# mohammadasim98/mv-ldm

Measured on AMD Instinct MI355X. Metric: denoised views/sec @ 256x256, 4 views, 50 DDIM steps, higher is better.
Workload: dtype bf16

## Files before the change

mv_ldm_amd/_build.py:

```python
from __future__ import annotations

import json
import os
import re
import subprocess
import sys
from concurrent.futures import ThreadPoolExecutor
from pathlib import Path

CSRC = Path(__file__).resolve().parent / "csrc"
LIB = CSRC / "libmvldm_hip.so"
SOURCES = ["api.cpp", "plan.cpp", "igemm.hip", "igemm_small.hip", "igemm_large.hip", "igemm_xl.hip", "igemm_halo.hip", "pack.hip", "attention.hip", "norm.hip", "misc.hip",
           "wgrad.hip", "attention_bwd.hip", "norm_bwd.hip", "train_misc.hip", "linear_pp.hip", "linear_pw.hip", "linear_ws.hip", "linear_rs.hip", "skinny.hip", "metrics.hip", "lpips.hip"]
HEADERS = [*sorted(CSRC.glob("*.h")), CSRC.parent.parent / "include" / "mvldm.h"]
FLAGS = ["--offload-arch=gfx950", "-O3", "-std=c++17", "-fPIC", "-ffp-contract=off", "-Wno-unused-result",
         "-Rpass-analysis=kernel-resource-usage"]
RES = CSRC / "kernel_resources.json"


def _hipcc() -> str:
    for c in (os.environ.get("HIPCC"), "/opt/rocm/bin/hipcc", "hipcc"):
        if c and (os.path.isabs(c) and os.path.exists(c) or not os.path.isabs(c)):
            return c
    raise RuntimeError("hipcc not found")


def _stale(target: Path, deps) -> bool:
    if not target.exists():
        return True
    t = target.stat().st_mtime
    return any(Path(d).stat().st_mtime > t for d in deps)


def build(force: bool = False, verbose: bool = False) -> Path:
    hipcc = _hipcc()
    flags = list(FLAGS)
    if os.environ.get("MVLDM_EXPERIMENTS") == "1":
        flags.append("-DMVLDM_EXPERIMENTS")
    objs, jobs = [], []
    for src in SOURCES:
        s = CSRC / src
        o = CSRC / (s.stem + ".o")
        objs.append(o)
        if force or _stale(o, [s, *HEADERS]):
            cmd = [hipcc, *flags, "-x", "hip", "-c", str(s), "-o", str(o)]
            jobs.append(cmd)
    if jobs:
        def run(cmd):
            if verbose:
                print(" ".join(cmd), flush=True)
            r = subprocess.run(cmd, capture_output=True, text=True)
            if r.returncode:
                raise RuntimeError(f"hipcc failed: {' '.join(cmd)}\n{r.stdout}\n{r.stderr}")
            Path(cmd[-1]).with_suffix(".res.json").write_text(json.dumps(_resources(r.stderr), indent=0))
        with ThreadPoolExecutor(max_workers=min(8, len(jobs))) as ex:
            list(ex.map(run, jobs))
    if force or jobs or _stale(LIB, objs):
        cmd = [hipcc, "--offload-arch=gfx950", "-shared", "-fPIC", "-o", str(LIB), *map(str, objs)]
        r = subprocess.run(cmd, capture_output=True, text=True)
        if r.returncode:
            raise RuntimeError(f"link failed:\n{r.stdout}\n{r.stderr}")
    parts = [o.with_suffix(".res.json") for o in objs]
    if all(q.exists() for q in parts) and (not RES.exists() or _stale(RES, parts)):
        merged = {}
        for q in parts:
            merged.update(json.loads(q.read_text()))
        RES.write_text(json.dumps(merged, indent=0, sort_keys=True))
    return LIB


_FIELDS = {"VGPRs": "vgpr", "AGPRs": "agpr", "TotalSGPRs": "sgpr", "ScratchSize [bytes/lane]": "scratch", "VGPRs Spill": "vgpr_spill",
           "Occupancy [waves/SIMD]": "waves_per_simd"}


def _resources(stderr: str) -> dict:
    out, cur = {}, None
    for line in stderr.splitlines():
        m = re.search(r"remark:\s+(.*?)\s*\[-Rpass-analysis", line)
        if not m:
            continue
        body = m.group(1)
        if body.startswith("Function Name:"):
            cur = out.setdefault(body.split(":", 1)[1].strip(), {})
        elif cur is not None and ":" in body:
            k, v = body.rsplit(":", 1)
            if k.strip() in _FIELDS and v.strip().lstrip("-").isdigit():
                cur[_FIELDS[k.strip()]] = int(v)
    return out


if __name__ == "__main__":
    print(build(force="--force" in sys.argv, verbose=True))
```

mv_ldm_amd/csrc/igemm.hip:

```cpp
#include <algorithm>
#include <cstdio>
#include <cstdlib>

#include "igemm_common.h"

namespace mvldm {

template <typename T> __global__ __launch_bounds__(256) void igemm_splitk_reduce(const IgemmParams p) {
    const bool geglu = p.epilogue == MVLDM_EPI_GEGLU;
    const size_t total = (size_t)p.M * p.n_dst;
    const size_t slab = (size_t)p.M * p.n_pad;
    for (size_t idx = (size_t)blockIdx.x * 256 + threadIdx.x; idx < total; idx += (size_t)gridDim.x * 256) {
        const int m = (int)(idx / p.n_dst), col = (int)(idx - (size_t)m * p.n_dst);
        float v;
        if (geglu) {
            const int nv = (col >> 5) * 64 + (col & 31), ng = nv + 32;
            float a = 0.f, g = 0.f;
            for (int s = 0; s < p.splitk; ++s) {
                a += p.ws[s * slab + (size_t)m * p.n_pad + nv];
                g += p.ws[s * slab + (size_t)m * p.n_pad + ng];
            }
            if (p.bias) { a += p.bias[col]; g += p.bias[p.n_dst + col]; }
            v = a * gelu_erf_fast(g);
        } else {
            float a = 0.f;
            for (int s = 0; s < p.splitk; ++s) a += p.ws[s * slab + (size_t)m * p.n_pad + col];
            if (p.bias) a += p.bias[col];
            if (p.row_bias) a += p.row_bias[(size_t)(m / p.hw_out) * p.row_bias_ld + col];
            if (p.epilogue == MVLDM_EPI_SILU) a = silu_f(a);
            else if (p.epilogue == MVLDM_EPI_GELU) a = gelu_erf_fast(a);
            v = a;
        }
        epilogue_store<T, true>(p, m, col, v);
    }
}

template <typename T> __global__ __launch_bounds__(256) void igemm_splitk_reduce_vec(const IgemmParams p) {
    const bool geglu = p.epilogue == MVLDM_EPI_GEGLU;
    const int cpr = p.n_dst / 8;
    const size_t total = (size_t)p.M * cpr;
    const size_t slab = (size_t)p.M * p.n_pad;
    for (size_t idx = (size_t)blockIdx.x * 256 + threadIdx.x; idx < total; idx += (size_t)gridDim.x * 256) {
        const int m = (int)(idx / cpr), col = (int)(idx - (size_t)m * cpr) * 8;
        const int nv = geglu ? (col >> 5) * 64 + (col & 31) : col;
        const float* w0 = p.ws + (size_t)m * p.n_pad + nv;
        float a[8], g[8];
#pragma unroll
        for (int e = 0; e < 8; ++e) a[e] = g[e] = 0.f;
        int s = 0;
        for (; s + 4 <= p.splitk; s += 4) {
            f32x4 lo[4], hi[4], gl[4], gh[4];
#pragma unroll
            for (int u = 0; u < 4; ++u) {
                lo[u] = *reinterpret_cast<const f32x4*>(w0 + (s + u) * slab);
                hi[u] = *reinterpret_cast<const f32x4*>(w0 + (s + u) * slab + 4);
                if (geglu) {
                    gl[u] = *reinterpret_cast<const f32x4*>(w0 + (s + u) * slab + 32);
                    gh[u] = *reinterpret_cast<const f32x4*>(w0 + (s + u) * slab + 36);
                }
            }
#pragma unroll
            for (int u = 0; u < 4; ++u) {
#pragma unroll
                for (int e = 0; e < 4; ++e) { a[e] += lo[u][e]; a[4 + e] += hi[u][e]; }
                if (geglu) {
#pragma unroll
                    for (int e = 0; e < 4; ++e) { g[e] += gl[u][e]; g[4 + e] += gh[u][e]; }
                }
            }
        }
        for (; s < p.splitk; ++s) {
            const f32x4 lo = *reinterpret_cast<const f32x4*>(w0 + s * slab), hi = *reinterpret_cast<const f32x4*>(w0 + s * slab + 4);
#pragma unroll
            for (int e = 0; e < 4; ++e) { a[e] += lo[e]; a[4 + e] += hi[e]; }
            if (geglu) {
                const f32x4 gl = *reinterpret_cast<const f32x4*>(w0 + s * slab + 32), gh = *reinterpret_cast<const f32x4*>(w0 + s * slab + 36);
#pragma unroll
                for (int e = 0; e < 4; ++e) { g[e] += gl[e]; g[4 + e] += gh[e]; }
            }
        }
        if (p.bias) {
#pragma unroll
            for (int e = 0; e < 8; ++e) a[e] += p.bias[col + e];
        }
        if (geglu) {
#pragma unroll
            for (int e = 0; e < 8; ++e) a[e] *= gelu_erf_fast(g[e] + (p.bias ? p.bias[p.n_dst + col + e] : 0.f));
        } else {
            if (p.row_bias) {
                const float* rb = p.row_bias + (size_t)(m / p.hw_out) * p.row_bias_ld + col;
#pragma unroll
                for (int e = 0; e < 8; ++e) a[e] += rb[e];
            }
            if (p.epilogue == MVLDM_EPI_SILU) {
#pragma unroll
                for (int e = 0; e < 8; ++e) a[e] = silu_f(a[e]);
            } else if (p.epilogue == MVLDM_EPI_GELU) {
#pragma unroll
                for (int e = 0; e < 8; ++e) a[e] = gelu_erf_fast(a[e]);
            }
        }
#pragma unroll
        for (int e = 0; e < 8; ++e) a[e] *= p.out_scale;
        if (p.residual) {
            const Chunk<T> rc = load_chunk<T>(reinterpret_cast<const T*>(p.residual) + (size_t)m * p.n_dst + col);
#pragma unroll
            for (int e = 0; e < 8; ++e) a[e] += rc.get(e);
        }
        size_t drow = (size_t)m;
        if (p.scatter) {
            const int img = m / p.hw_out, rem = m - img * p.hw_out;
            const int i = rem / p.w_out, j = rem - i * p.w_out;
            drow = ((size_t)img * (2 * p.h_out) + 2 * i + p.ph_y) * (size_t)(2 * p.w_out) + 2 * j + p.ph_x;
        }
        Chunk<T> oc;
#pragma unroll
        for (int e = 0; e < 8; ++e) oc.set(e, a[e]);
        store_chunk<T>(reinterpret_cast<T*>(p.dst) + drow * p.dst_ld + col, oc);
    }
}

static int env_int(const char* name, int dflt) { return knob_int(name, dflt); }
static const int kEnvTarget = env_int("MVLDM_IGEMM_TARGET", 0);
static const int kEnvSync = env_int("MVLDM_IGEMM_SYNC", 0);
static const int kEnvPx = env_int("MVLDM_IGEMM_PX", 0);
static const int kEnvNoStage = env_int("MVLDM_IGEMM_NOSTAGE", 0);
#ifdef MVLDM_EXPERIMENTS
static const int kEnvFake = env_int("MVLDM_IGEMM_FAKE", 0);
#else
static constexpr int kEnvFake = 0;
#endif

static thread_local int t_force_sync = 0;

static int launch_igemm(const IgemmParams& p, int tile, int act_dtype, hipStream_t s) {
    if (tile >= 1 && tile <= 5) return igemm_launch_small(p, tile, act_dtype, s);
    if (tile >= 6 && tile <= 8) return igemm_launch_large(p, tile, act_dtype, s);
    if (tile == 9 || tile == 10 || tile == 18) return igemm_launch_xl(p, tile, act_dtype, s);
    if (tile == 11 || tile == 17) return igemm_launch_halo(p, tile, act_dtype, s);
    return set_error(MVLDM_ERR_ARG, "igemm: bad tile %d", tile);
}


static void choose_config(const mvldm_igemm_desc& d, int M, int k_tiles, int& tile, int& splitk, size_t ws_bytes) {
    const int target = kEnvTarget ? kEnvTarget : 512;
    if (tile == 0) {
        const bool can10 = d.act_dtype != MVLDM_F32 && d.k_order == 1 && d.dst_dtype != MVLDM_F32 && d.n_pad % 320 == 0 &&
                           d.epilogue != MVLDM_EPI_GEGLU && d.upsample != 1 && d.n_out % 8 == 0 && (d.dst_ld <= 0 || d.dst_ld % 8 == 0) &&
                           !(d.ksize == 3 && d.src1);
        const int wgs10 = cdiv(M, 256) * (d.n_pad / 320);
        const double eff10 = (double)wgs10 / (256.0 * cdiv(wgs10, 256));
        if (can10 && (wgs10 >= 1024 || (wgs10 >= 512 && (eff10 >= 0.9 || d.ksize == 1)))) tile = 10;
        else if (M <= 32) tile = 5;
        else if (M <= 64) tile = 4;
        else if (d.ksize >= 2) tile = cdiv(M, 256) * cdiv(d.n_pad, 128) >= 300 ? 7 : 2;
        else if (d.n_pad >= 768 && d.act_dtype != MVLDM_F32 && d.k_order == 1 && d.dst_dtype != MVLDM_F32 &&
                 cdiv(M, 256) * cdiv(d.n_pad, 256) >= 1024)
            tile = 9;
        else if (d.k_pad >= 1024 && d.n_pad >= 1024 && cdiv(M, 128) * cdiv(d.n_pad, 256) >= 300) tile = 8;
        else tile = d.n_pad < 640 ? 2 : 3;
    }
    const int tm = cdiv(M, kTiles[tile].bm), tn = cdiv(d.n_pad, kTiles[tile].bn);
    if (splitk == 0) {
        splitk = 1;
        const int wgs = tm * tn;
        if (wgs < target) splitk = std::min(std::max(k_tiles / 4, 1), cdiv(target, wgs));
        if (d.workspace == nullptr) splitk = 1;
        while (splitk > 1 && (size_t)splitk * M * d.n_pad * sizeof(float) > ws_bytes) --splitk;
    }
    splitk = std::max(1, std::min(splitk, k_tiles));
}

static int fill_params(const mvldm_igemm_desc& d, IgemmParams& p, int& tile) {
    const int epc = d.act_dtype == MVLDM_F32 ? 4 : 8;
    const int bk = d.act_dtype == MVLDM_F32 ? 32 : 64;
    MVLDM_REQUIRE(d.src0 && d.weight && d.dst, "igemm: null pointer");
    const bool phase = d.upsample >= 2;
    MVLDM_REQUIRE(d.upsample >= 0 && d.upsample <= 5, "igemm: upsample %d", d.upsample);
    MVLDM_REQUIRE(phase ? (d.ksize == 2 && d.stride == 1 && d.h_out == d.h_in && d.w_out == d.w_in && !d.src1 && !d.residual &&
                           !d.row_bias && d.act_dtype != MVLDM_F32 && d.dst_dtype == d.act_dtype && d.k_order == 1)
                        : (d.ksize == 1 || d.ksize == 3),
                  "igemm: ksize %d / upsample %d", d.ksize, d.upsample);
    MVLDM_REQUIRE(d.stride == 1 || d.stride == 2, "igemm: stride %d", d.stride);
    MVLDM_REQUIRE(d.c0 % epc == 0 && d.c1 % epc == 0 && d.c0 > 0, "igemm: channels (%d,%d) must be multiples of %d", d.c0, d.c1, epc);
    MVLDM_REQUIRE((d.c1 == 0) == (d.src1 == nullptr), "igemm: src1/c1 mismatch");
    MVLDM_REQUIRE(d.k_pad % bk == 0 && d.k_pad >= d.ksize * d.ksize * (d.c0 + d.c1), "igemm: k_pad %d", d.k_pad);
    MVLDM_REQUIRE(d.n_pad % 64 == 0 && d.n_pad >= d.n_out, "igemm: n_pad %d (n_out %d)", d.n_pad, d.n_out);
    MVLDM_REQUIRE(d.dst_dtype == d.act_dtype || d.dst_dtype == MVLDM_F32, "igemm: dst dtype");
    if (d.epilogue == MVLDM_EPI_GEGLU)
        MVLDM_REQUIRE(d.n_out % 64 == 0 && !d.row_bias, "igemm: GEGLU needs n_out %% 64 == 0");
    p.src0 = d.src0; p.src1 = d.src1; p.weight = d.weight; p.bias = d.bias; p.row_bias = d.row_bias;
    p.residual = d.residual; p.dst = d.dst; p.ws = d.workspace;
    p.c0 = d.c0; p.c1 = d.c1; p.ctot = d.c0 + d.c1;
    p.n_img = d.n_img; p.h_in = d.h_in; p.w_in = d.w_in; p.h_out = d.h_out; p.w_out = d.w_out;
    p.hw_out = d.h_out * d.w_out;
    p.ksize = d.ksize; p.stride = d.stride; p.pad = d.pad; p.upsample = phase ? 0 : d.upsample; p.taps = d.ksize * d.ksize;
    p.scatter = phase; p.ph_y = phase ? (d.upsample - 2) >> 1 : 0; p.ph_x = phase ? (d.upsample - 2) & 1 : 0;
    p.ty0 = phase ? p.ph_y - 1 : -d.pad; p.tx0 = phase ? p.ph_x - 1 : -d.pad;
    p.cy = phase ? 1 - p.ph_y : d.ksize / 2; p.cx = phase ? 1 - p.ph_x : d.ksize / 2;
    p.M = d.n_img * p.hw_out; p.n_out = d.n_out; p.n_pad = d.n_pad; p.k_pad = d.k_pad;
    p.n_dst = d.epilogue == MVLDM_EPI_GEGLU ? d.n_out / 2 : d.n_out;
    p.rb_vec = d.row_bias && ((uintptr_t)d.row_bias % 16 == 0) && d.row_bias_ld % 4 == 0;
    p.bias_vec = d.bias && ((uintptr_t)d.bias % 16 == 0);
    p.row_bias_ld = d.row_bias_ld; p.epilogue = d.epilogue; p.dst_f32 = d.dst_dtype == MVLDM_F32;
    p.out_scale = d.out_scale;
    p.dst_ld = d.dst_ld > 0 ? d.dst_ld : p.n_dst;
    MVLDM_REQUIRE(p.dst_ld >= p.n_dst, "igemm: dst_ld %d < n_dst %d", p.dst_ld, p.n_dst);
    p.k_tiles = d.k_pad / bk;
    tile = d.tile & 63;
    t_force_sync = (d.tile >> 12) & 1;
    const int force_px = (d.tile >> 8) & 15;
    int splitk = d.splitk;
    MVLDM_REQUIRE(((tile >= 0 && tile <= kNumTiles) || tile == 17 || deep_tile(tile)) && splitk >= 0, "igemm: tile/splitk");
    choose_config(d, p.M, p.k_tiles, tile, splitk, d.workspace_bytes);
    if (splitk > 1)
        MVLDM_REQUIRE(d.workspace && (size_t)splitk * p.M * d.n_pad * sizeof(float) <= d.workspace_bytes,
                      "igemm: split-K workspace too small");
    const double es = 2.0;
    const double b0 = (double)d.n_img * d.h_in * d.w_in * d.c0 * es, b1 = (double)d.n_img * d.h_in * d.w_in * d.c1 * es;
    const double bw = (double)d.n_pad * d.k_pad * es;
    p.use_bl = d.act_dtype != MVLDM_F32 && d.k_order == 1 && !t_force_sync && !kEnvSync &&
               b0 < 4.0e9 && b1 < 4.0e9 && bw < 4.0e9;
    if (d.act_dtype != MVLDM_F32 && d.k_order == 1 && !t_force_sync && !kEnvSync && !p.use_bl) {
        static bool warned = false;
        if (!warned) {
            warned = true;
            fprintf(stderr, "[mvldm] igemm: operand of %.2f GB exceeds the 4 GB range of the fast 16-bit loop; using the slower "
                            "64-bit-address loop (split the batch to avoid this)\n", std::max(std::max(b0, b1), bw) / 1e9);
        }
    }
    p.src0_bytes = (unsigned)b0; p.src1_bytes = (unsigned)b1; p.w_bytes = (unsigned)bw;
    p.fake = kEnvFake;
    p.nt_store = stream_stores((size_t)p.M * (size_t)p.n_dst * (p.dst_f32 || d.act_dtype == MVLDM_F32 ? 4 : 2));
    if (kEnvFake & 1) p.src0_bytes = p.src1_bytes = 0;
    if (kEnvFake & 2) p.w_bytes = 0;
    if (tile >= 6 && !p.use_bl) tile = 2;
    if (deep_tile(tile) && d.upsample) tile = 2;
    p.splitk = splitk;
    if (p.use_bl) {
        const int cbs = p.k_tiles / p.taps;
        const int per = cdiv(cbs, std::min(splitk, cbs));
        p.k_tiles_per_split = per * p.taps;
        p.splitk = cdiv(cbs, per);
    } else {
        p.k_tiles_per_split = cdiv(p.k_tiles, splitk);
        p.splitk = cdiv(p.k_tiles, p.k_tiles_per_split);
    }
    p.stage_epi = d.act_dtype != MVLDM_F32 && !kEnvNoStage && (p.splitk > 1 || (!p.dst_f32 && p.n_dst % 8 == 0 && p.dst_ld % 8 == 0));
    if (tile >= 9 && tile <= 10 && (!p.stage_epi || (tile == 10 && d.epilogue == MVLDM_EPI_GEGLU))) tile = 7;
    if (tile == 11 && !(p.use_bl && p.stage_epi && p.splitk == 1 && d.ksize == 3 && d.stride == 1 && d.pad == 1 && !d.upsample &&
                        d.h_out == d.h_in && d.w_out == d.w_in && halo_rows_for(d.w_in) <= 384 && halo_smem(d.w_in) <= 160 * 1024))
        tile = 7;
    if (tile == 17 && !(p.use_bl && p.stage_epi && p.splitk == 1 && d.ksize == 3 && d.stride == 1 && d.pad == 1 && !d.upsample && d.c1 == 0 &&
                        d.h_out == d.h_in && d.w_out == d.w_in && d.epilogue != MVLDM_EPI_GEGLU && halow_smem(d.w_in) <= 160 * 1024))
        tile = 7;
    if (phase) {
        MVLDM_REQUIRE(p.use_bl && p.stage_epi, "igemm: 2x2 phase conv needs the lean 16-bit loop and an 8-aligned 16-bit output");
        if (tile != 7 && tile != 10) tile = 2;
    }
    if (p.use_bl && d.upsample == 1 && tile != 7) tile = 2;
    if (p.use_bl && d.upsample != 1) {
        const int hc = (d.h_out - 1) * d.stride + p.ty0 + p.cy, wc = (d.w_out - 1) * d.stride + p.tx0 + p.cx;
        MVLDM_REQUIRE(p.ty0 + p.cy >= 0 && p.tx0 + p.cx >= 0 && hc < d.h_in && wc < d.w_in,
                      "igemm: conv geometry (pad %d, stride %d) not supported", d.pad, d.stride);
    }
    p.tiles_m = cdiv(p.M, kTiles[tile].bm);
    p.tiles_n = cdiv(d.n_pad, kTiles[tile].bn);
    p.korder = d.k_order;
    if (d.k_order)
        MVLDM_REQUIRE(d.k_order == 1 && p.ctot % bk == 0 && d.c0 % bk == 0 && d.k_pad == p.taps * p.ctot,
                      "igemm: k_order 1 needs channel counts (%d,%d) multiples of %d", d.c0, d.c1, bk);
    {
        const double a_bytes = (double)d.n_img * d.h_in * d.w_in * p.ctot, w_bytes = (double)d.n_pad * d.k_pad;
        double best = 1e300;
        for (int px = 1; px <= 8; px *= 2) {
            const int py = 8 / px;
            const int sm = cdiv(p.tiles_m, px), sn = cdiv(p.tiles_n, py);
            const double waste = (double)(8 * sm * sn) / ((double)p.tiles_m * p.tiles_n);
            const double cost = (py * a_bytes + px * w_bytes) * waste * waste;
            if (cost < best) { best = cost; p.px = px; p.sub_m = sm; p.sub_n = sn; }
        }
        p.m_fast = w_bytes >= a_bytes;
        const int fpx = force_px ? force_px : kEnvPx;
        if (fpx > 0 && fpx <= 8 && (8 % fpx) == 0) {
            p.px = fpx; p.sub_m = cdiv(p.tiles_m, p.px); p.sub_n = cdiv(p.tiles_n, 8 / p.px);
        }
        p.grp_m = p.grp_n = 1;
        static const int kGroup = knob_int("MVLDM_IGEMM_GROUP", -1);
        if (kGroup != 0 && ((tile >= 7 && tile <= 10) || tile == 17) && p.sub_m * p.sub_n > 32) {
            const double ax = a_bytes / p.px, wx = w_bytes / (8 / p.px);
            double bestc = 1e300;
            for (int gm = 1; gm <= 32; gm *= 2) {
                if (kGroup > 0 && gm != kGroup) continue;
                const int gme = std::min(gm, p.sub_m), gne = std::min(32 / gm, p.sub_n);
                const double c = ax * cdiv(p.sub_n, gne) + wx * cdiv(p.sub_m, gme);
                if (c < bestc) { bestc = c; p.grp_m = gme; p.grp_n = gne; }
            }
        }
    }
    return MVLDM_OK;
}

int linear_pp_run(const mvldm_igemm_desc& d, hipStream_t s);
int linear_pw_run(const mvldm_igemm_desc& d, hipStream_t s);
int linear_ws_run(const mvldm_igemm_desc& d, hipStream_t s);
int skinny_run(const mvldm_igemm_desc& d, hipStream_t s);
int linear_rs_run(const mvldm_igemm_desc& d, hipStream_t s);

int igemm_run(const mvldm_igemm_desc& d, hipStream_t s) {
    IgemmParams p;
    int tile = 0;
    if (d.n_img == 0 || d.h_out == 0 || d.w_out == 0) return MVLDM_OK;
    const int req = d.tile & 63;
    if (req == 15) return skinny_run(d, s);
    if (req == 12 || req == 13 || req == 14 || req == 19) {
        MVLDM_REQUIRE(d.src0 && d.weight && d.dst, "igemm: null pointer");
        return req == 12 ? linear_pp_run(d, s) : req == 13 ? linear_pw_run(d, s) : req == 14 ? linear_ws_run(d, s) : linear_rs_run(d, s);
    }
    MVLDM_REQUIRE(d.k_order != 2, "igemm: the fragment-order pack (k_order 2) is read by tile 15 only");
    int rc = fill_params(d, p, tile);
    if (rc) return rc;
    if (p.M == 0) return MVLDM_OK;
    rc = dispatch_dtype(d.act_dtype, [&](auto t) {
        using T = decltype(t);
        int r = launch_igemm(p, tile, Elt<T>::DT, s);
        if (r) return r;
        if (p.splitk > 1) {
            if constexpr (sizeof(T) == 2) {
                if (!p.dst_f32 && p.n_dst % 8 == 0 && p.dst_ld % 8 == 0 && ((uintptr_t)p.ws % 16) == 0 &&
                    (!p.residual || ((uintptr_t)p.residual % 16) == 0) && ((uintptr_t)p.dst % 16) == 0) {
                    const size_t chunks = (size_t)p.M * (p.n_dst / 8);
                    hipLaunchKernelGGL(igemm_splitk_reduce_vec<T>, dim3((unsigned)std::min<size_t>((chunks + 255) / 256, 4096)), dim3(256), 0, s, p);
                    return check_launch();
                }
            }
            const size_t total = (size_t)p.M * p.n_dst;
            const int blocks = (int)std::min<size_t>((total + 255) / 256, 4096);
            hipLaunchKernelGGL(igemm_splitk_reduce<T>, dim3(blocks), dim3(256), 0, s, p);
            return check_launch();
        }
        return (int)MVLDM_OK;
    });
    return rc;
}

}

using namespace mvldm;

extern "C" int mvldm_igemm_fwd(const mvldm_igemm_desc* d, mvldm_stream_t stream) {
    MVLDM_REQUIRE(d != nullptr, "igemm: null desc");
    return igemm_run(*d, (hipStream_t)stream);
}

extern "C" size_t mvldm_igemm_workspace_bytes(const mvldm_igemm_desc* d) {
    if (!d) return 0;
    const size_t M = (size_t)d->n_img * d->h_out * d->w_out;
    return (size_t)16 * M * d->n_pad * sizeof(float);
}
```

mv_ldm_amd/csrc/linear_pw.hip:

```cpp
#include <cstdlib>

#include "linear_common.h"

namespace mvldm {

struct LinPWParams {
    const void* a; const void* a1; const void* w; const float* bias; const void* residual; void* dst;
    int M, K, c0, c1, kt0, n_out, n_pad, n_dst, dst_ld, k_steps;
    int tiles_m, tiles_n, m_per;
    int gm, gn, nbn, wgx;
    int nt_store, touch;
    int spread;
    float out_scale;
    unsigned a_bytes, a1_bytes, w_bytes, bias_bytes, res_bytes, dst_bytes;
    unsigned* trace; int trace_blk, trace_wave, trace_stagger;
};

#ifdef MVLDM_PW_TRACE
#define PW_STAMP() if (tr_on && tr_n < 190) { reinterpret_cast<unsigned*>(smem + G::SLAB + 1280)[tr_n++] = (unsigned)__builtin_readcyclecounter(); }
#else
#define PW_STAMP()
#endif

#ifdef MVLDM_EXPERIMENTS
static const int kPwFake = knob_int("MVLDM_PW_FAKE", 0);
#else
static constexpr int kPwFake = 0;
#endif
#ifdef MVLDM_EXPERIMENTS_NOGELU
#define PW_GELU(x) (x)
#else
#define PW_GELU(x) gelu_erf_16(x)
#endif

constexpr int PW_BM = 256, PW_NW = 8;
#ifndef PW_SP3
#define PW_SP3 4
#define PW_SP0 3
#define PW_SP1 2
#endif

template <int TN> struct PwGeo {
    static constexpr int BN = 64 * TN;
    static constexpr int A_SLOT = PW_BM * 128, W_SLOT = BN * 128, STAGE = A_SLOT + W_SLOT;
    static constexpr int A_IT = PW_BM / 8 / PW_NW;
    static constexpr int W_IT = BN / 8 / PW_NW;
    static constexpr int P = A_IT + W_IT;
    static constexpr int Q0 = PW_SP3 < P ? PW_SP3 : P, Q1 = Q0 + PW_SP0 < P ? Q0 + PW_SP0 : P, Q2 = Q1 + PW_SP1 < P ? Q1 + PW_SP1 : P;
    static constexpr int RING = 2 * STAGE;
    static constexpr int SLAB = RING;
    static constexpr int SMEM = SLAB + 2048;
};

struct PwAddr {
    unsigned a0, a1;
    unsigned w;
    int m0, n0;
    bool valid;
};

template <int TN, int LO = 0, int HI = 1 << 20>
__device__ __forceinline__ void pw_issue_a(const LinPWParams& p, char* smem, int slot, int wave, int lane, int ks, const PwAddr& ad) {
    using G = PwGeo<TN>;
    const bool second = ks >= p.kt0;
    const void* abase = second ? p.a1 : p.a;
    const unsigned abytes = second ? p.a1_bytes : p.a_bytes;
    const int c = second ? p.c1 : p.c0;
    const __amdgpu_buffer_rsrc_t ra = __builtin_amdgcn_make_buffer_rsrc(const_cast<void*>(abase), 0, abytes, 0x00020000);
    const int soff = (second ? ks - p.kt0 : ks) * 128;
    char* stage = smem + slot * G::STAGE;
    const unsigned v = second ? ad.a1 : ad.a0;
    const int row = wave * 8 + (lane >> 3);
#pragma unroll
    for (int it = (LO > 0 ? LO : 0); it < (HI < G::A_IT ? HI : G::A_IT); ++it) {
        const unsigned off = (ad.valid && ad.m0 + row + 64 * it < p.M) ? v : kBufOob;
        __builtin_amdgcn_raw_ptr_buffer_load_lds(ra, (__attribute__((address_space(3))) void*)(stage + (wave + PW_NW * it) * 1024), 16, off,
                                                 soff + it * 128 * c, 0, 0);
    }
}
template <int TN, int LO = 0, int HI = 1 << 20>
__device__ __forceinline__ void pw_issue_w(const LinPWParams& p, char* smem, int slot, int wave, int ks, const PwAddr& ad) {
    using G = PwGeo<TN>;
    const __amdgpu_buffer_rsrc_t rw = __builtin_amdgcn_make_buffer_rsrc(const_cast<void*>(p.w), 0, p.w_bytes, 0x00020000);
    const int soff = ks * 128;
    char* stage = smem + slot * G::STAGE + G::A_SLOT;
#pragma unroll
    for (int it = (LO > 0 ? LO : 0); it < (HI < G::W_IT ? HI : G::W_IT); ++it) {
        const unsigned off = (ad.valid && ad.n0 + 64 * it < p.n_pad) ? ad.w : kBufOob;
        __builtin_amdgcn_raw_ptr_buffer_load_lds(rw, (__attribute__((address_space(3))) void*)(stage + (wave + PW_NW * it) * 1024), 16, off,
                                                 soff + it * 128 * p.K, 0, 0);
    }
}

template <int TN, int LO, int HI>
__device__ __forceinline__ void pw_issue_group(const LinPWParams& p, char* smem, int slot, int wave, int lane, int ks, const PwAddr& ad) {
    using G = PwGeo<TN>;
    if constexpr (LO < HI && LO < G::A_IT) pw_issue_a<TN, LO, HI>(p, smem, slot, wave, lane, ks, ad);
    if constexpr (LO < HI && HI > G::A_IT) pw_issue_w<TN, LO - G::A_IT, HI - G::A_IT>(p, smem, slot, wave, ks, ad);
}

template <int TN>
__device__ __forceinline__ void pw_touch_a(const LinPWParams& p, char* smem, int wave, int lane, int tm, int ks, bool valid) {
    using G = PwGeo<TN>;
    const bool second = ks >= p.kt0;
    const void* abase = second ? p.a1 : p.a;
    const unsigned abytes = second ? p.a1_bytes : p.a_bytes;
    const int c = second ? p.c1 : p.c0;
    const __amdgpu_buffer_rsrc_t ra = __builtin_amdgcn_make_buffer_rsrc(const_cast<void*>(abase), 0, abytes, 0x00020000);
    const int m = tm * PW_BM + wave * 32 + (lane >> 1);
    const unsigned off = (valid && m < p.M) ? ((unsigned)m * (unsigned)c * 2u + (unsigned)(lane & 1) * 64u) : kBufOob;
    __builtin_amdgcn_raw_ptr_buffer_load_lds(ra, (__attribute__((address_space(3))) void*)(smem + G::SLAB + 1792), 4, off,
                                             (second ? ks - p.kt0 : ks) * 128, 0, 0);
}

template <int TN>
__device__ __forceinline__ void pw_offsets(const LinPWParams& p, bool valid, int tm, int tn, int wave, int lane, PwAddr& ad) {
    using G = PwGeo<TN>;
    const int slot = lane & 7, rsub = lane >> 3;
    const int row = wave * 8 + rsub;
    const unsigned chunk = (unsigned)((slot ^ ((row >> 1) & 7)) * 8);
    const int m = tm * PW_BM + row, n = tn * G::BN + row;
    ad.a0 = ((unsigned)m * (unsigned)p.c0 + chunk) * 2u;
    ad.a1 = ((unsigned)m * (unsigned)p.c1 + chunk) * 2u;
    ad.w = ((unsigned)n * (unsigned)p.K + chunk) * 2u;
    ad.m0 = tm * PW_BM;
    ad.n0 = tn * G::BN;
    ad.valid = valid;
}

template <int TN>
__device__ __forceinline__ unsigned pw_bias_off(const LinPWParams& p, bool geglu, bool valid, int tn, int t) {
    using G = PwGeo<TN>;
    const int pc = tn * G::BN + 4 * t;
    int oc = pc;
    if (geglu) {
        const int blk = pc >> 5, w = pc & 31;
        oc = ((blk & 1) ? p.n_dst : 0) + (blk >> 1) * 32 + w;
    }
    return (valid && 4 * t < G::BN && pc < p.n_out) ? (unsigned)oc * 4u : kBufOob;
}

template <bool NT>
__device__ __forceinline__ void pw_store2(const u32x4& rdst, const u32x4& d0, unsigned o0, const u32x4& d1, unsigned o1) {
    if constexpr (NT)
        asm volatile("s_nop 4\n\tbuffer_store_dwordx4 %0, %1, %4, 0 offen nt\n\tbuffer_store_dwordx4 %2, %3, %4, 0 offen nt\n\ts_nop 2"
                     ::"v"(d0), "v"(o0), "v"(d1), "v"(o1), "s"(rdst) : "memory");
    else
        asm volatile("s_nop 4\n\tbuffer_store_dwordx4 %0, %1, %4, 0 offen\n\tbuffer_store_dwordx4 %2, %3, %4, 0 offen\n\ts_nop 2"
                     ::"v"(d0), "v"(o0), "v"(d1), "v"(o1), "s"(rdst) : "memory");
}

template <int CTRL> __device__ __forceinline__ u32x4 pw_qperm(const u32x4& v) {
    u32x4 r;
#pragma unroll
    for (int c = 0; c < 4; ++c) r[c] = (unsigned)__builtin_amdgcn_update_dpp(0, (int)v[c], CTRL, 0xF, 0xF, true);
    return r;
}
__device__ __forceinline__ u32x4 pw_sel(bool take_a, const u32x4& a, const u32x4& b) {
    u32x4 r;
#pragma unroll
    for (int c = 0; c < 4; ++c) r[c] = take_a ? a[c] : b[c];
    return r;
}
__device__ __forceinline__ void pw_quad_transpose(u32x4& c0, u32x4& c1, u32x4& c2, u32x4& c3, bool odd, bool upper) {
    constexpr int X1 = 0xB1, X2 = 0x4E;
    const u32x4 x0 = pw_sel(odd, pw_qperm<X1>(c1), c0), x1 = pw_sel(odd, c1, pw_qperm<X1>(c0));
    const u32x4 x2 = pw_sel(odd, pw_qperm<X1>(c3), c2), x3 = pw_sel(odd, c3, pw_qperm<X1>(c2));
    c0 = pw_sel(upper, pw_qperm<X2>(x2), x0);
    c2 = pw_sel(upper, x2, pw_qperm<X2>(x0));
    c1 = pw_sel(upper, pw_qperm<X2>(x3), x1);
    c3 = pw_sel(upper, x3, pw_qperm<X2>(x1));
}
__device__ __forceinline__ unsigned pw_line_off(int M, int tm, int wm, int i, int j, int half, int l31, int hi, int col0, int ld, int n_dst) {
    const int t = 2 * (j & 1) + half, k = l31 & 3;
    const int m = tm * PW_BM + wm * 64 + i * 32 + (l31 & ~3) + t;
    const int col = col0 + 32 * (j & ~1) + 8 * (2 * k + hi);
    return (m < M && col < n_dst) ? ((unsigned)m * (unsigned)ld + (unsigned)col) * 2u : kBufOob;
}

template <typename T, int TN, int EPI, bool RES, bool NT>
__global__ __launch_bounds__(512) void linear_pw_kernel(const LinPWParams p) {
    using G = PwGeo<TN>;
    using Frag = typename LinMma<T>::Frag;
    constexpr bool GEGLU = EPI == MVLDM_EPI_GEGLU;
    static_assert(!GEGLU || TN % 2 == 0, "GEGLU pairs value / gate blocks inside a wave tile");
    static_assert(!(GEGLU && RES), "no caller");
    constexpr int NOUT = GEGLU ? TN / 2 : TN;
    extern __shared__ __attribute__((aligned(16))) char smem[];
    const int tid = threadIdx.x, lane = tid & 63;
    const int wave = __builtin_amdgcn_readfirstlane(tid >> 6);
    const int wm = wave >> 1, wn = wave & 1;
    const int hi = lane >> 5, l31 = lane & 31;
    const int prm = lin_perm(l31);

    const int xcd = blockIdx.x & 7, lid = blockIdx.x >> 3;
    const int m_lo = xcd * p.m_per, m_cnt = min(p.tiles_m, m_lo + p.m_per) - m_lo;
    LinTileIter<LinPWParams> cur, nxt, iss;
    cur.set(p, 0, lid, m_lo, m_cnt);
    if (!cur.valid) return;
    nxt.set(p, cur.r + 1, lid, m_lo, m_cnt);
    iss = cur;

    u32x4 rdst;
    rdst[0] = (unsigned)(uintptr_t)p.dst; rdst[1] = (unsigned)((uintptr_t)p.dst >> 32) & 0xFFFFu; rdst[2] = p.dst_bytes; rdst[3] = 0x00020000u;

    const int a_off = (wm * 64 + l31) * 128 + ((hi ^ ((l31 >> 1) & 7)) << 4);
    const int w_off = G::A_SLOT + (wn * 32 * TN + prm) * 128 + ((hi ^ ((prm >> 1) & 7)) << 4);

    f32x16 acc[2][TN];
    PwAddr ad;
    int ks_i = 1;
    const int kT = p.k_steps;

#ifdef MVLDM_PW_TRACE
    for (int i = 0; i < (lid & 3) * p.trace_stagger; ++i) __builtin_amdgcn_s_sleep(8);
#endif
    {
        pw_offsets<TN>(p, true, cur.tm, cur.tn, wave, lane, ad);
#pragma unroll
        for (int g = 0; g < 2; ++g) {
            pw_issue_a<TN>(p, smem, g, wave, lane, g, ad);
            pw_issue_w<TN>(p, smem, g, wave, g, ad);
        }
        const u32x4 b = lin_load_bias<G::BN>(p, GEGLU, true, cur.tn, tid);
        __builtin_amdgcn_s_waitcnt(waitcnt_vmcnt(0));
        if (4 * tid < G::BN) *reinterpret_cast<u32x4*>(smem + G::SLAB + tid * 16) = b;
    }
    int rs = 0;
#ifdef MVLDM_PW_TRACE
    const bool tr_on = p.trace && (int)blockIdx.x == p.trace_blk && wave == p.trace_wave;
    int tr_n = 0;
#endif

#define PW_SUB(ca_, cw_, na_, nw_, NEXT_, nslot_, nkk_, MODE_, SPN_)                                              \
    {                                                                                                             \
        const char* st_ = smem + (nslot_) * G::STAGE;                                                             \
        const int ao_ = a_off ^ ((nkk_) << 5), wo_ = w_off ^ ((nkk_) << 5);                                       \
        if (NEXT_) {                                                                                              \
            na_[0] = lin_frag<T>(st_ + ao_);                                                                      \
            na_[1] = lin_frag<T>(st_ + ao_ + 4096);                                                               \
            nw_[0] = lin_frag<T>(st_ + wo_);                                                                      \
        }                                                                                                         \
        _Pragma("unroll") for (int j = 0; j < TN; ++j) {                                                          \
            __builtin_amdgcn_sched_barrier(0);                                                                    \
            acc[0][j] = LinMma<T>::mma(cw_[j], ca_[0], acc[0][j]);                                                \
            acc[1][j] = LinMma<T>::mma(cw_[j], ca_[1], acc[1][j]);                                                \
            if (NEXT_ && j + 1 < TN) nw_[j + 1] = lin_frag<T>(st_ + wo_ + (j + 1) * 4096);                        \
            if ((MODE_) == 1 && j == 0) {                                                                         \
                if (++ks_i == kT) {                                                                               \
                    ks_i = 0;                                                                                     \
                    iss.set(p, iss.r + 1, lid, m_lo, m_cnt);                                                  \
                    pw_offsets<TN>(p, iss.valid, iss.tm, iss.tn, wave, lane, ad);                                 \
                }                                                                                                 \
                if (SPN_) pw_issue_group<TN, 0, G::Q0>(p, smem, rs, wave, lane, ks_i, ad);                        \
                else pw_issue_a<TN>(p, smem, rs, wave, lane, ks_i, ad);                                           \
            }                                                                                                     \
            if ((MODE_) == 1 && j == 2 && !(SPN_)) pw_issue_w<TN>(p, smem, rs, wave, ks_i, ad);                   \
            if ((MODE_) == 2 && j == 1 && pend) pw_issue_group<TN, G::Q0, G::Q1>(p, smem, rs ^ 1, wave, lane, ks_i, ad); \
            if ((MODE_) == 3 && j == 1 && pend) pw_issue_group<TN, G::Q1, G::Q2>(p, smem, rs ^ 1, wave, lane, ks_i, ad); \
            if ((MODE_) == 4 && j == 1 && pend) pw_issue_group<TN, G::Q2, G::P>(p, smem, rs ^ 1, wave, lane, ks_i, ad);  \
        }                                                                                                         \
        __builtin_amdgcn_sched_barrier(0);                                                                        \
    }
#define PW_STEP(LAST_, WAIT_, TOUCH_, SPN_)                                                                       \
    {                                                                                                             \
        PW_STAMP()                                                                                                \
        if ((TOUCH_) && p.touch) {                                                                                \
             \
            const int kt_ = ks_t + PW_TOUCH_AHEAD;                                                                \
            const bool own_ = kt_ < kT;                                                                           \
            pw_touch_a<TN>(p, smem, wave, lane, __builtin_amdgcn_readfirstlane(own_ ? cur.tm : nxt.tm),           \
                           __builtin_amdgcn_readfirstlane(own_ ? kt_ : kt_ - kT), own_ || nxt.valid);             \
        }                                                                                                         \
        PW_SUB(fa0, fw0, fa1, fw1, true, rs, 1, 2, false)                                                         \
        PW_SUB(fa1, fw1, fa0, fw0, true, rs, 2, 3, false)                                                         \
        PW_SUB(fa0, fw0, fa1, fw1, true, rs, 3, 4, false)                                                         \
        PW_STAMP()                                                                                                \
        if ((TOUCH_) && p.touch) __builtin_amdgcn_s_waitcnt(kWaitStep1);                                          \
        else __builtin_amdgcn_s_waitcnt(WAIT_);                                                                   \
        PW_STAMP()                                                                                                \
        __builtin_amdgcn_s_barrier();                                                                             \
        PW_STAMP()                                                                                                \
        {                                                                                                         \
            const bool spn_ = (SPN_);                                                                             \
            PW_SUB(fa1, fw1, fa0, fw0, !(LAST_), rs ^ 1, 0, 1, spn_)                                              \
            pend = spn_;                                                                                          \
        }                                                                                                         \
        rs ^= 1;                                                                                                  \
    }
    bool pend = false;
    const bool sp = p.spread && !p.touch && kT >= 4;
    Frag fa0[2], fw0[TN], fa1[2], fw1[TN];
    constexpr int kWaitLds = 0xC07F;
    constexpr int kWaitFirst = waitcnt_vmcnt(4 * NOUT) & ~0x0F00;
    constexpr int kWaitStepT = waitcnt_vmcnt(0) & ~0x0F00;
    constexpr int kWaitStep1 = waitcnt_vmcnt(1) & ~0x0F00;
    constexpr int PW_TOUCH_AHEAD = 4;

    for (; cur.valid; cur = nxt, nxt.set(p, nxt.r + 1, lid, m_lo, m_cnt)) {
        __builtin_amdgcn_s_barrier();
        {
            const float* slab = reinterpret_cast<const float*>(smem + G::SLAB) + wn * 32 * TN + 8 * hi;
#pragma unroll
            for (int j = 0; j < TN; ++j)
#pragma unroll
                for (int a = 0; a < 4; ++a) {
                    const f32x4 b = *reinterpret_cast<const f32x4*>(slab + 32 * j + 16 * (a >> 1) + 4 * (a & 1));
#pragma unroll
                    for (int e = 0; e < 4; ++e) { acc[0][j][4 * a + e] = b[e]; acc[1][j][4 * a + e] = b[e]; }
                }
        }
        {
            const char* st0 = smem + rs * G::STAGE;
#pragma unroll
            for (int i = 0; i < 2; ++i) fa0[i] = lin_frag<T>(st0 + a_off + i * 4096);
#pragma unroll
            for (int j = 0; j < TN; ++j) fw0[j] = lin_frag<T>(st0 + w_off + j * 4096);
        }
        { const int ks_t = 0; PW_STEP(false, kWaitFirst, false, sp) }
#pragma unroll 1
        for (int ks_t = 1; ks_t < kT - 1; ++ks_t) PW_STEP(false, kWaitStepT, true, sp && ks_t + 2 < kT)
        u32x4 bnext;
        {
            u32x4 rbias;
            rbias[0] = (unsigned)(uintptr_t)p.bias; rbias[1] = (unsigned)((uintptr_t)p.bias >> 32) & 0xFFFFu; rbias[2] = p.bias_bytes; rbias[3] = 0x00020000u;
            const unsigned boff = pw_bias_off<TN>(p, GEGLU, nxt.valid, nxt.tn, tid);
            asm volatile("s_nop 4\n\tbuffer_load_dwordx4 %0, %1, %2, 0 offen" : "=v"(bnext) : "v"(boff), "s"(rbias));
        }
        { const int ks_t = 0; PW_STEP(true, kWaitLds, false, false) }
        PW_STAMP()
        {
            const int col0 = GEGLU ? (cur.tn * G::BN + wn * 32 * TN) >> 1 : cur.tn * G::BN + wn * 32 * TN;
            const bool q_odd = (l31 & 1) != 0, q_upper = (l31 & 2) != 0;
            unsigned row_dst[2], row_res[2];
#pragma unroll
            for (int i = 0; i < 2; ++i) {
                const int m = cur.tm * PW_BM + wm * 64 + i * 32 + l31;
                row_dst[i] = m < p.M ? (unsigned)m * (unsigned)p.dst_ld * 2u : kLinRowNone;
                row_res[i] = m < p.M ? (unsigned)m * (unsigned)p.n_dst * 2u : kLinRowNone;
            }
            u32x4 out[2][NOUT][2];
            if constexpr (RES) {
                constexpr int NB = 2 * TN;
                u32x4 rres;
                rres[0] = (unsigned)(uintptr_t)p.residual; rres[1] = (unsigned)((uintptr_t)p.residual >> 32) & 0xFFFFu; rres[2] = p.res_bytes; rres[3] = 0x00020000u;
                u32x4 r[NB][2];
#define PW_RES_OFFS(b_)                                                                                                         \
        const bool pair_ = (((b_) % TN) | 1) < TN;                                                                              \
        const unsigned o0_ = pair_ ? pw_line_off(p.M, cur.tm, wm, (b_) / TN, (b_) % TN, 0, l31, hi, col0, p.n_dst, p.n_dst)     \
                                   : lin_off(row_res[(b_) / TN], col0 + 32 * ((b_) % TN) + 8 * hi, p.n_dst);                    \
        const unsigned o1_ = pair_ ? pw_line_off(p.M, cur.tm, wm, (b_) / TN, (b_) % TN, 1, l31, hi, col0, p.n_dst, p.n_dst)     \
                                   : lin_off(row_res[(b_) / TN], col0 + 32 * ((b_) % TN) + 16 + 8 * hi, p.n_dst);
#define PW_RES_ISSUE(b_)                                                                                                        \
    if constexpr ((b_) < NB) {                                                                                                  \
        PW_RES_OFFS(b_)                                                                                                         \
        asm volatile("s_nop 4\n\tbuffer_load_dwordx4 %0, %2, %4, 0 offen\n\tbuffer_load_dwordx4 %1, %3, %4, 0 offen"             \
                     : "=&v"(r[(b_) < NB ? (b_) : 0][0]), "=&v"(r[(b_) < NB ? (b_) : 0][1]) : "v"(o0_), "v"(o1_), "s"(rres));   \
    }
#define PW_RES_BLOCK(b_)                                                                                                        \
    if constexpr ((b_) < NB) {                                                                                                  \
        constexpr int i_ = (b_) / TN, j_ = (b_) % TN;                                                                           \
        constexpr int left_ = NB - 1 - (b_) < PW_D - 1 ? NB - 1 - (b_) : PW_D - 1;                                              \
        if constexpr ((b_) == 0) {                                                                                              \
            asm volatile("s_waitcnt vmcnt(%3)" : "+v"(r[0][0]), "+v"(r[0][1]), "+v"(bnext) : "n"(2 * left_));                  \
            if (4 * tid < G::BN) *reinterpret_cast<u32x4*>(smem + G::SLAB + tid * 16) = bnext;                                  \
        } else {                                                                                                                \
            asm volatile("s_waitcnt vmcnt(%2)" : "+v"(r[(b_) < NB ? (b_) : 0][0]), "+v"(r[(b_) < NB ? (b_) : 0][1]) : "n"(2 * left_)); \
        }                                                                                                                       \
        constexpr bool paired_ = (j_ | 1) < TN;                                                                                 \
        if constexpr (!paired_) {                                                                                               \
            float c_[16];                                                                                                       \
            _Pragma("unroll") for (int k = 0; k < 16; ++k) c_[k] = acc[i_][j_][k];                                              \
            lin_pack<T, true>(c_, p.out_scale, r[(b_) < NB ? (b_) : 0], out[i_][j_]);                                           \
        } else if constexpr ((j_ & 1) == 1) {                                                                                   \
                \
            constexpr int bp_ = (b_) > 0 ? (b_) - 1 : 0;                                                                        \
            pw_quad_transpose(r[bp_][0], r[bp_][1], r[(b_) < NB ? (b_) : 0][0], r[(b_) < NB ? (b_) : 0][1], q_odd, q_upper);    \
            float c_[16];                                                                                                       \
            _Pragma("unroll") for (int k = 0; k < 16; ++k) c_[k] = acc[i_][j_ - 1][k];                                          \
            lin_pack<T, true>(c_, p.out_scale, r[bp_], out[i_][j_ - 1]);                                                        \
            _Pragma("unroll") for (int k = 0; k < 16; ++k) c_[k] = acc[i_][j_][k];                                              \
            lin_pack<T, true>(c_, p.out_scale, r[(b_) < NB ? (b_) : 0], out[i_][j_]);                                           \
            pw_quad_transpose(out[i_][j_ - 1][0], out[i_][j_ - 1][1], out[i_][j_][0], out[i_][j_][1], q_odd, q_upper);          \
        }                                                                                                                       \
        PW_RES_ISSUE((b_) + PW_D)                                                                                               \
    }
                constexpr int PW_D = 4;
                PW_RES_ISSUE(0) PW_RES_ISSUE(1) PW_RES_ISSUE(2) PW_RES_ISSUE(3)
                PW_RES_BLOCK(0) PW_RES_BLOCK(1) PW_RES_BLOCK(2) PW_RES_BLOCK(3) PW_RES_BLOCK(4)
                PW_RES_BLOCK(5) PW_RES_BLOCK(6) PW_RES_BLOCK(7) PW_RES_BLOCK(8) PW_RES_BLOCK(9)
                static_assert(NB <= 10, "blocks listed above");
#undef PW_RES_ISSUE
#undef PW_RES_BLOCK
            } else {
                asm volatile("s_waitcnt vmcnt(%1)" : "+v"(bnext) : "n"(G::P));
                if (4 * tid < G::BN) *reinterpret_cast<u32x4*>(smem + G::SLAB + tid * 16) = bnext;
#pragma unroll
                for (int i = 0; i < 2; ++i)
#pragma unroll
                    for (int j = 0; j < NOUT; ++j) {
                        float c[16];
                        if constexpr (GEGLU) {
#pragma unroll
                            for (int k = 0; k < 16; ++k) c[k] = acc[i][2 * j][k] * PW_GELU(acc[i][2 * j + 1][k]);
                        } else {
#pragma unroll
                            for (int k = 0; k < 16; ++k) c[k] = acc[i][j][k];
                        }
                        const u32x4 none[2] = {u32x4{0u, 0u, 0u, 0u}, u32x4{0u, 0u, 0u, 0u}};
                        lin_pack<T, false>(c, p.out_scale, none, out[i][j]);
                        if ((j & 1) == 1) pw_quad_transpose(out[i][j - 1][0], out[i][j - 1][1], out[i][j][0], out[i][j][1], q_odd, q_upper);
                    }
            }
#pragma unroll
            for (int i = 0; i < 2; ++i)
#pragma unroll
                for (int j = 0; j < NOUT; ++j)
                    if ((j | 1) < NOUT)
                        pw_store2<NT>(rdst, out[i][j][0], pw_line_off(p.M, cur.tm, wm, i, j, 0, l31, hi, col0, p.dst_ld, p.n_dst), out[i][j][1],
                                      pw_line_off(p.M, cur.tm, wm, i, j, 1, l31, hi, col0, p.dst_ld, p.n_dst));
                    else
                        pw_store2<NT>(rdst, out[i][j][0], lin_off(row_dst[i], col0 + 32 * j + 8 * hi, p.n_dst), out[i][j][1],
                                      lin_off(row_dst[i], col0 + 32 * j + 16 + 8 * hi, p.n_dst));
        }
    }
#ifdef MVLDM_PW_TRACE
    if (tr_on) {
        PW_STAMP()
        asm volatile("s_waitcnt lgkmcnt(0)" ::: "memory");
        for (int i = lane; i < 192; i += 64) p.trace[i] = i < tr_n ? reinterpret_cast<const unsigned*>(smem + G::SLAB + 1280)[i] : 0u;
    }
#endif
#undef PW_SUB
#undef PW_STEP
}

bool linear_pw_applicable(const mvldm_igemm_desc& d) {
    if (d.act_dtype == MVLDM_F32 || d.dst_dtype != d.act_dtype) return false;
    if (d.ksize != 1 || d.stride != 1 || d.upsample != 0 || d.row_bias || d.k_order != 1 || d.splitk > 1) return false;
    if (d.h_in != d.h_out || d.w_in != d.w_out || d.pad != 0) return false;
    if (d.epilogue != MVLDM_EPI_NONE && d.epilogue != MVLDM_EPI_GEGLU) return false;
    if (d.epilogue != MVLDM_EPI_NONE && d.residual) return false;
    const int n_dst = d.epilogue == MVLDM_EPI_GEGLU ? d.n_out / 2 : d.n_out;
    const int dst_ld = d.dst_ld > 0 ? d.dst_ld : n_dst;
    if ((d.c1 == 0) != (d.src1 == nullptr) || d.c0 % 64 || d.c1 % 64 || d.c0 + d.c1 < 320 || d.k_pad != d.c0 + d.c1 || d.n_out % 8 || n_dst % 8 || dst_ld % 8 || dst_ld < n_dst) return false;
    if (d.epilogue == MVLDM_EPI_GEGLU && d.n_out % 64) return false;
    if (d.bias && ((uintptr_t)d.bias % 16)) return false;
    if (((uintptr_t)d.dst % 16) || (d.residual && ((uintptr_t)d.residual % 16))) return false;
    const double m = (double)d.n_img * d.h_out * d.w_out;
    return m * d.c0 * 2.0 < 4.0e9 && m * d.c1 * 2.0 < 4.0e9 && (double)d.n_pad * d.k_pad * 2.0 < 4.0e9 && m * dst_ld * 2.0 < 4.0e9 && m * n_dst * 2.0 < 4.0e9;
}

template <typename T, int TN, int EPI, bool RES, bool NT> static int linear_pw_launch1(const LinPWParams& p, int grid, hipStream_t s) {
    static std::atomic<uint64_t> done{0};
    if (int rc0 = ensure_dyn_smem(reinterpret_cast<const void*>(linear_pw_kernel<T, TN, EPI, RES, NT>), PwGeo<TN>::SMEM, done)) return rc0;
    hipLaunchKernelGGL((linear_pw_kernel<T, TN, EPI, RES, NT>), dim3(grid), dim3(512), PwGeo<TN>::SMEM, s, p);
    return check_launch();
}
template <typename T, int TN, int EPI, bool RES> static int linear_pw_launch(const LinPWParams& p, int grid, hipStream_t s) {
    return p.nt_store ? linear_pw_launch1<T, TN, EPI, RES, true>(p, grid, s) : linear_pw_launch1<T, TN, EPI, RES, false>(p, grid, s);
}

int linear_pw_run(const mvldm_igemm_desc& d, hipStream_t s) {
    MVLDM_REQUIRE(linear_pw_applicable(d), "igemm: tile 13 (persistent wide Linear) does not apply to this problem");
    LinPWParams p;
    lin_fill_params2(p, d, kPwFake);
    p.k_steps = p.K / 64;
    const bool geglu = d.epilogue == MVLDM_EPI_GEGLU;
    static const int kForceTn = knob_int("MVLDM_PW_TN", 0);
    const int cu_x = std::max(1, cu_count() / 8);
    p.tiles_m = (p.M + PW_BM - 1) / PW_BM;
    p.m_per = (p.tiles_m + 7) / 8;
    auto launch_cost = [&](int tnb) {
        const int tiles = p.m_per * ((d.n_pad + 64 * tnb - 1) / (64 * tnb));
        const int wg = std::min(cu_x, tiles);
        return (double)((tiles + wg - 1) / wg) * tnb;
    };
    int tn_blocks = (!geglu && d.n_pad % 320 == 0) ? 5 : 4;
    if (tn_blocks == 5 && launch_cost(4) < 0.95 * launch_cost(5)) tn_blocks = 4;
    if (kForceTn == 4 || (kForceTn == 5 && !geglu)) tn_blocks = kForceTn;
    const int bn = 64 * tn_blocks;
    p.tiles_n = (d.n_pad + bn - 1) / bn;
    static const int kNt = knob_int("MVLDM_STREAM_STORES", 0);
    p.nt_store = kNt == 1;
    p.spread = !((d.tile >> 14) & 1);
    p.touch = (d.tile >> 13) & 1;
    p.trace = nullptr; p.trace_blk = 0; p.trace_wave = 0; p.trace_stagger = 0;
#ifdef MVLDM_PW_TRACE
    if (const char* tp = getenv("MVLDM_PW_TRACE_PTR")) {
        p.trace = reinterpret_cast<unsigned*>(strtoull(tp, nullptr, 16));
        p.trace_blk = getenv("MVLDM_PW_TRACE_BLK") ? atoi(getenv("MVLDM_PW_TRACE_BLK")) : 8;
        p.trace_wave = getenv("MVLDM_PW_TRACE_WAVE") ? atoi(getenv("MVLDM_PW_TRACE_WAVE")) : 0;
        p.trace_stagger = getenv("MVLDM_PW_STAGGER") ? atoi(getenv("MVLDM_PW_STAGGER")) : 0;
    }
#endif
    p.wgx = std::min(cu_x, p.m_per * p.tiles_n);
    lin_block_shape(p, 256.0 * p.K * 2.0, (double)bn * p.K * 2.0);
    static const int kForceGm = knob_int("MVLDM_PW_GM", 0);
    if (kForceGm > 0) { p.gm = std::min(std::min(kForceGm, p.wgx), p.m_per); p.gn = std::max(1, std::min(p.wgx / p.gm, p.tiles_n)); }
    p.nbn = (p.tiles_n + p.gn - 1) / p.gn;
    const int grid = 8 * p.wgx;
    const bool res = d.residual != nullptr;
    return dispatch_dtype(d.act_dtype, [&](auto t) -> int {
        using T = decltype(t);
        if constexpr (sizeof(T) == 2) {
            if (geglu) return linear_pw_launch<T, 4, MVLDM_EPI_GEGLU, false>(p, grid, s);
            if (tn_blocks == 5) return res ? linear_pw_launch<T, 5, MVLDM_EPI_NONE, true>(p, grid, s) : linear_pw_launch<T, 5, MVLDM_EPI_NONE, false>(p, grid, s);
            return res ? linear_pw_launch<T, 4, MVLDM_EPI_NONE, true>(p, grid, s) : linear_pw_launch<T, 4, MVLDM_EPI_NONE, false>(p, grid, s);
        } else {
            return set_error(MVLDM_ERR_ARG, "igemm: tile 13 needs a 16-bit activation type");
        }
    });
}

}
```

mv_ldm_amd/plan.py:

```python
from __future__ import annotations

import ctypes as C
import json
import os
import sys
from dataclasses import dataclass
from typing import List, Optional

import torch

from . import _lib as L
from .ops import PackedWeight, conv_out_hw, dt, igemm_desc, ptr, use_skinny


def _PIN_TILE() -> int:
    v = os.environ.get("MVLDM_IGEMM_TILE")
    return int(v) if v else 0


@dataclass
class OpMeta:
    name: str
    kind: int
    flops: float = 0.0
    bytes: float = 0.0


class Builder:
    def __init__(self, device, dtype: torch.dtype, record: bool = False, splitk_ws_bytes: int = 256 << 20):
        self.device, self.dtype, self.record = torch.device(device), dtype, record
        self.ops: List[L.Op] = []
        self.meta: List[OpMeta] = []
        self.keep: list = []
        self._pool: dict = {}
        self._ws = None
        self._ws_bytes = splitk_ws_bytes
        self._gn_ws = None
        self._scope: List[str] = []
        self._lane = 0
        self._lane_ws: dict = {}
        self._deferred: Optional[list] = None
        self.skinny = True
        self._skinny_pw: dict = {}

    def empty(self, *shape, dtype=None) -> torch.Tensor:
        dtype = dtype or self.dtype
        if self.record:
            nbytes = int(torch.Size(shape).numel()) * torch.empty(0, dtype=dtype).element_size()
            free = self._pool.get(nbytes)
            if free:
                base = free.pop()
                return base.view(dtype).view(*shape)
        t = torch.empty(*shape, dtype=dtype, device=self.device)
        if self.record:
            self.keep.append(t)
            self.__dict__.setdefault("_own_ptrs", set()).add(t.data_ptr())
        return t

    def free(self, t: Optional[torch.Tensor]):
        if t is None or not self.record:
            return
        base = t.reshape(-1).view(torch.uint8)
        if self._deferred is not None:
            self._deferred.append(base)
            return
        self._pool.setdefault(base.numel(), []).append(base)

    class _Parallel:

        def __init__(self, b):
            self.b, self.n = b, 0

        def __enter__(self):
            assert self.b._deferred is None, "parallel groups do not nest"
            self.b._marker(L.OP_PAR_BEGIN, "par_begin")
            self.b._deferred = []
            return self

        def lane(self):
            if self.n:
                self.b._marker(L.OP_PAR_NEXT, "par_next")
            self.b._lane = self.n
            self.n += 1

        def __exit__(self, *a):
            b = self.b
            b._marker(L.OP_PAR_END, "par_end")
            b._lane = 0
            deferred, b._deferred = b._deferred, None
            for base in deferred:
                b._pool.setdefault(base.numel(), []).append(base)

    def parallel(self):
        return Builder._Parallel(self)

    def _marker(self, kind: int, name: str):
        op = L.Op()
        op.kind = kind
        self._emit(op, name)

    def splitk_ws(self) -> torch.Tensor:
        if self._lane:
            ws = self._lane_ws.get(("splitk", self._lane))
            if ws is None:
                ws = torch.empty(min(self._ws_bytes, 64 << 20), dtype=torch.uint8, device=self.device)
                self._lane_ws[("splitk", self._lane)] = ws
                self.keep.append(ws)
            return ws
        if self._ws is None:
            self._ws = torch.empty(self._ws_bytes, dtype=torch.uint8, device=self.device)
            self.keep.append(self._ws)
        return self._ws

    def gn_ws(self, n_img: int, groups: int) -> torch.Tensor:
        need = n_img * L.GN_MAX_CHUNKS * groups * 16
        if self._lane:
            ws = self._lane_ws.get(("gn", self._lane))
            if ws is None or ws.numel() < need:
                ws = torch.empty(max(need, 1 << 16), dtype=torch.uint8, device=self.device)
                self._lane_ws[("gn", self._lane)] = ws
                self.keep.append(ws)
            return ws
        if self._gn_ws is None or self._gn_ws.numel() < need:
            self._gn_ws = torch.empty(max(need, 1 << 16), dtype=torch.uint8, device=self.device)
            self.keep.append(self._gn_ws)
        return self._gn_ws

    class _Scope:
        def __init__(self, b, name):
            self.b, self.name = b, name

        def __enter__(self):
            self.b._scope.append(self.name)

        def __exit__(self, *a):
            self.b._scope.pop()

    def scope(self, name: str):
        return Builder._Scope(self, name)

    def _emit(self, op: L.Op, name: str, flops=0.0, nbytes=0.0, refs=()):
        if self.record:
            op.tag = len(self.ops)
            self.ops.append(op)
            self.meta.append(OpMeta("/".join(self._scope + [name]), op.kind, flops, nbytes))
            self.keep.extend(r for r in refs if r is not None)
        else:
            L.check(L.load().mvldm_op_run(C.byref(op), torch.cuda.current_stream().cuda_stream))

    def conv(self, x, pw: PackedWeight, bias=None, *, x2=None, stride=1, pad=None, upsample=False, row_bias=None,
             residual=None, epilogue=L.EPI_NONE, out_dtype=None, out_scale=1.0, out=None, name="conv", splitk=0, tile=0):
        n, h, w, c0 = x.shape
        c1 = 0 if x2 is None else x2.shape[-1]
        pad = (pw.ksize // 2) if pad is None else pad
        ho, wo = conv_out_hw(h, w, pw.ksize, stride, pad, upsample)
        n_dst = pw.n_out // 2 if epilogue == L.EPI_GEGLU else pw.n_out
        if out is None:
            out = self.empty(n, ho, wo, n_dst, dtype=out_dtype or x.dtype)
        ws = self.splitk_ws() if splitk != 1 else None
        if tile == 0 and _PIN_TILE() and x.dtype != torch.float32 and pw.k_order == 1:
            tile, splitk = _PIN_TILE(), 1
        m = n * ho * wo
        k_real = pw.ksize * pw.ksize * (c0 + c1)
        es = x.element_size()
        nbytes = (pw.n_out * k_real + n * h * w * (c0 + c1)) * es + m * n_dst * out.element_size() \
            + (m * n_dst * es if residual is not None else 0)
        self._igemm(x, x2, pw, bias, row_bias, residual, out, ws, name, 2.0 * m * pw.n_out * k_real, nbytes, h_out=ho, w_out=wo,
                    stride=stride, pad=pad, upsample=upsample, epilogue=epilogue, out_scale=out_scale, splitk=splitk, tile=tile)
        return out

    def _igemm(self, x, x2, pw, bias, row_bias, residual, out, ws, name, flops, nbytes, *, h_out, w_out, tile=0, **desc):
        n, h, w, c0 = x.shape
        c1 = 0 if x2 is None else x2.shape[-1]
        op = L.Op()
        op.kind = L.OP_IGEMM
        d = igemm_desc(x, x2, pw, out, n_img=n, h_in=h, w_in=w, h_out=h_out, w_out=w_out, bias=bias, row_bias=row_bias,
                       residual=residual, ws=ws, tile=tile, into=op.u.igemm, **desc)
        m = n * h_out * w_out
        can_sk = tile == 0 and self.skinny and skinny_candidate(pw, m, c0, c1, d.upsample, x.dtype) \
            and x.is_cuda and L.load().mvldm_igemm_skinny_config(C.byref(d)) > 0
        if can_sk and skinny_rule(m, pw.n_pad):
            tile = d.tile = 15
            use_skinny(d, pw)
        elif can_sk and self.record:
            self._skinny_pw[len(self.ops)] = pw
        if self.record:
            own = self.__dict__.get("_own_ptrs", ())
            self.__dict__.setdefault("_tune_srcs", {})[len(self.ops)] = tuple(t if (t is not None and t.data_ptr() in own) else None
                                                                              for t in (x, x2))
        self._emit(op, name, flops, nbytes, (x, x2, pw.data, pw._skinny if (tile & 63) == 15 else None, bias, row_bias, residual, out))

    def small_launch(self, rows: int, n_out: int) -> bool:
        limit = int(os.environ.get("MVLDM_PAR_ROWS", "0"))
        return self.record and rows * max(n_out, 1) <= limit * 640 and limit > 0

    def conv_upsample_phases(self, x, pws, bias=None, name="upsample"):
        n, h, w, c0 = x.shape
        out = self.empty(n, 2 * h, 2 * w, pws[0].n_out, dtype=x.dtype)
        lanes = self.parallel() if self.small_launch(n * h * w, pws[0].n_out) else None
        if lanes is not None:
            lanes.__enter__()
        for phase, pw in enumerate(pws):
            if lanes is not None:
                lanes.lane()
            self._phase_conv(x, pw, bias, out, phase, name)
        if lanes is not None:
            lanes.__exit__(None, None, None)
        return out

    def _phase_conv(self, x, pw, bias, out, phase, name, tile=0, splitk=0):
        n, h, w, c0 = x.shape
        ws = self.splitk_ws()
        assert pw.ksize == 2 and pw.k_order == 1 and c0 == pw.c_pad
        m = n * h * w
        es = x.element_size()
        nbytes = (pw.n_out * 4 * c0 + (m * c0 if phase == 0 else 0)) * es + m * pw.n_out * es
        self._igemm(x, None, pw, bias, None, None, out, ws, f"{name}.p{phase}", 2.0 * m * pw.n_out * 4 * c0, nbytes, h_out=h, w_out=w,
                    stride=1, pad=0, upsample=2 + phase, splitk=splitk, tile=tile)

    def linear(self, x, pw: PackedWeight, bias=None, *, residual=None, epilogue=L.EPI_NONE, out_dtype=None, out=None,
               name="linear", row_bias=None):
        rows, c = x.shape
        y = self.conv(x.view(rows, 1, 1, c), pw, bias, residual=None if residual is None else residual.view(rows, 1, 1, -1),
                      epilogue=epilogue, out_dtype=out_dtype, out=None if out is None else out.view(rows, 1, 1, -1),
                      name=name, row_bias=row_bias)
        return y.view(rows, -1)

    def groupnorm(self, x, gamma, beta, groups, eps, silu, x2=None, name="groupnorm", stats_out=None):
        n, c0 = x.shape[0], x.shape[-1]
        c1 = 0 if x2 is None else x2.shape[-1]
        hw = x.numel() // (n * c0)
        y = self.empty(*x.shape[:-1], c0 + c1, dtype=x.dtype)
        op = L.Op()
        op.kind = L.OP_GROUPNORM
        g = op.u.groupnorm
        g.x, g.x1, g.y, g.gamma, g.beta = ptr(x), ptr(x2), ptr(y), ptr(gamma), ptr(beta)
        g.stats_ws = self.gn_ws(n, groups).data_ptr()
        g.n_img, g.hw, g.c0, g.c1, g.groups, g.silu, g.dtype, g.eps = n, hw, c0, c1, groups, int(silu), dt(x), eps
        g.stats_out = ptr(stats_out)
        passes = L.load().mvldm_groupnorm_passes(n, hw, c0 + c1, groups, dt(x))
        self._emit(op, name, 0.0, float(passes) * y.numel() * y.element_size(), (x, x2, y, gamma, beta, stats_out))
        return y

    def layernorm(self, x, gamma, beta, eps=1e-5, name="layernorm"):
        c = x.shape[-1]
        rows = x.numel() // c
        y = self.empty(*x.shape, dtype=x.dtype)
        op = L.Op()
        op.kind = L.OP_LAYERNORM
        l = op.u.layernorm
        l.x, l.y, l.gamma, l.beta, l.rows, l.c, l.dtype, l.eps = ptr(x), ptr(y), ptr(gamma), ptr(beta), rows, c, dt(x), eps
        self._emit(op, name, 0.0, 2.0 * y.numel() * y.element_size(), (x, y, gamma, beta))
        return y

    def attention(self, q, k, v, heads, head_dim, seg, q_lens, kv_lens, scale=None, name="attention", lse=None, out=None):
        assert q.stride(1) == 1 and k.stride(1) == 1 and v.stride(1) == 1
        if out is None:
            out = self.empty(q.shape[0], heads * head_dim, dtype=q.dtype)
        op = L.Op()
        op.kind = L.OP_ATTENTION
        a = op.u.attention
        a.q, a.k, a.v, a.out, a.seg = ptr(q), ptr(k), ptr(v), ptr(out), ptr(seg)
        a.ld_q, a.ld_k, a.ld_v, a.ld_o = q.stride(0), k.stride(0), v.stride(0), out.stride(0)
        a.heads, a.head_dim, a.n_seg, a.max_q_len, a.dtype = heads, head_dim, seg.shape[0], max(q_lens), dt(q)
        a.scale = head_dim ** -0.5 if scale is None else scale
        a.lse, a.lse_ld = ptr(lse), (0 if lse is None else lse.stride(0))
        pairs = sum(ql * kl for ql, kl in zip(q_lens, kv_lens))
        es = q.element_size()
        nbytes = (sum(q_lens) * 2 + sum(kv_lens) * 2) * heads * head_dim * es
        self._emit(op, name, 4.0 * pairs * heads * head_dim, nbytes, (q, k, v, out, seg, lse))
        return out

    def attention_merge(self, oa, lse_a, ob, lse_b, out, a_img, b_img, out_img, tokens, heads, head_dim, name="attention_merge"):
        n = a_img.numel()
        assert b_img.numel() == n and out_img.numel() == n and all(i.dtype == torch.int32 for i in (a_img, b_img, out_img))
        assert lse_a.dtype == torch.float32 and lse_b.dtype == torch.float32 and oa.dtype == ob.dtype == out.dtype
        op = L.Op()
        op.kind = L.OP_ATTN_MERGE
        m = op.u.attn_merge
        m.oa, m.ob, m.out, m.lse_a, m.lse_b, m.a_img, m.b_img, m.out_img = ptr(oa), ptr(ob), ptr(out), ptr(lse_a), ptr(lse_b), ptr(a_img), ptr(b_img), ptr(out_img)
        m.n_img, m.tokens, m.heads, m.head_dim = n, tokens, heads, head_dim
        m.ld_a, m.ld_b, m.ld_o, m.lse_ld_a, m.lse_ld_b, m.dtype = oa.stride(0), ob.stride(0), out.stride(0), lse_a.stride(0), lse_b.stride(0), dt(oa)
        self._emit(op, name, 0.0, 3.0 * n * tokens * heads * head_dim * oa.element_size(), (oa, lse_a, ob, lse_b, out, a_img, b_img, out_img))

    def timestep_embed(self, timesteps, freqs, dim, flip, dtype, name="time_proj"):
        out = self.empty(timesteps.numel(), dim, dtype=dtype)
        op = L.Op()
        op.kind = L.OP_TIMESTEP_EMBED
        t = op.u.temb
        t.timesteps, t.freqs, t.out, t.n, t.dim, t.flip, t.dst_dtype = ptr(timesteps), ptr(freqs), ptr(out), timesteps.numel(), dim, int(flip), dt(out)
        self._emit(op, name, 0.0, out.numel() * out.element_size(), (timesteps, freqs, out))
        return out

    def eltwise(self, x, op_code, out_dtype=None, name="eltwise"):
        y = self.empty(*x.shape, dtype=out_dtype or x.dtype)
        op = L.Op()
        op.kind = L.OP_ELTWISE
        e = op.u.eltwise
        e.x, e.y, e.n, e.op, e.src_dtype, e.dst_dtype = ptr(x), ptr(y), x.numel(), op_code, dt(x), dt(y)
        self._emit(op, name, 0.0, x.numel() * (x.element_size() + y.element_size()), (x, y))
        return y

    def ddim_step(self, eps, x_t, x_next, cond_img, uncond_img, cfg_scale, coef, step_ptr, unet_in, name="ddim_cfg_step",
                  clip_range: float = 0.0):
        n_tgt, h, w, c = x_t.shape
        op = L.Op()
        op.kind = L.OP_DDIM_STEP
        d = op.u.ddim
        d.eps, d.x_t, d.x_next, d.cond_img, d.uncond_img = ptr(eps), ptr(x_t), ptr(x_next), ptr(cond_img), ptr(uncond_img)
        d.coef, d.step_ptr, d.unet_in = ptr(coef), ptr(step_ptr), ptr(unet_in)
        d.n_tgt, d.hw, d.c, d.cfg_scale = n_tgt, h * w, c, cfg_scale
        d.unet_in_c = 0 if unet_in is None else unet_in.shape[-1]
        d.unet_in_dtype = L.F32 if unet_in is None else dt(unet_in)
        d.n_steps, d.clip_range = coef.shape[0], clip_range
        self._emit(op, name, 0.0, 5.0 * x_t.numel() * 4, (eps, x_t, x_next, cond_img, uncond_img, coef, step_ptr, unet_in))
        return x_next

    def ddim_advance(self, step_ptr, t_table, timesteps, tgt_rows, name="ddim_advance"):
        op = L.Op()
        op.kind = L.OP_DDIM_ADVANCE
        a = op.u.advance
        a.step_ptr, a.t_table, a.timesteps, a.tgt_rows = ptr(step_ptr), ptr(t_table), ptr(timesteps), ptr(tgt_rows)
        a.n_steps, a.n_rows = t_table.numel(), 0 if tgt_rows is None else tgt_rows.numel()
        self._emit(op, name, 0.0, 0.0, (step_ptr, t_table, timesteps, tgt_rows))

    def memcpy(self, dst, src, name="memcpy"):
        assert dst.is_contiguous() and src.is_contiguous() and dst.numel() * dst.element_size() == src.numel() * src.element_size()
        op = L.Op()
        op.kind = L.OP_MEMCPY
        op.u.memcpy_.src, op.u.memcpy_.dst, op.u.memcpy_.bytes = ptr(src), ptr(dst), src.numel() * src.element_size()
        self._emit(op, name, 0.0, 2.0 * src.numel() * src.element_size(), (dst, src))

    def gather_rows(self, src, dst, src_index=None, dst_index=None, n_rows=None, name="gather_rows"):
        idx = src_index if src_index is not None else dst_index
        n = int(n_rows if n_rows is not None else (idx.numel() if idx is not None else dst.shape[0]))
        row_bytes = dst[0].numel() * dst.element_size()
        assert src[0].numel() * src.element_size() == row_bytes and row_bytes % 16 == 0 and dst.is_contiguous() and src.is_contiguous()
        assert all(i is None or (i.dtype == torch.int32 and i.numel() == n) for i in (src_index, dst_index))
        assert (src_index is not None or src.shape[0] >= n) and (dst_index is not None or dst.shape[0] >= n)
        op = L.Op()
        op.kind = L.OP_GATHER_ROWS
        g = op.u.gather
        g.src, g.dst, g.src_index, g.dst_index, g.row_bytes, g.n_rows = ptr(src), ptr(dst), ptr(src_index), ptr(dst_index), row_bytes, n
        self._emit(op, name, 0.0, 2.0 * n * row_bytes, (src, dst, src_index, dst_index))

    def nhwc_to_nchw(self, src, dst, c=None, c_off=0, scale=1.0, shift=0.0, clamp01=False, name="nhwc_to_nchw"):
        n, h, w, sc = src.shape
        op = L.Op()
        op.kind = L.OP_NHWC_TO_NCHW
        l = op.u.layout
        l.src, l.dst, l.n_img, l.c, l.hw, l.other_c, l.other_c_off, l.dtype = ptr(src), ptr(dst), n, c or sc, h * w, sc, c_off, dt(src)
        l.clamp01, l.scale, l.shift = int(clamp01), scale, shift
        self._emit(op, name, 0.0, src.numel() * src.element_size() + dst.numel() * 4, (src, dst))
        return dst

    def nchw_to_nhwc(self, src, dst, c_off=0, scale=1.0, shift=0.0, img_map=None, name="nchw_to_nhwc"):
        n, c, h, w = src.shape
        op = L.Op()
        op.kind = L.OP_NCHW_TO_NHWC
        l = op.u.layout
        l.src, l.dst, l.n_img, l.c, l.hw, l.other_c, l.other_c_off, l.dtype = ptr(src), ptr(dst), n, c, h * w, dst.shape[-1], c_off, dt(dst)
        l.scale, l.shift, l.img_map = scale, shift, ptr(img_map)
        self._emit(op, name, 0.0, src.numel() * 4 + src.numel() * dst.element_size(), (src, dst, img_map))
        return dst

    def ray_encode(self, extr, intr, h, w, out_nhwc, c_off, img_map=None, out_nchw=None, name="ray_encode", mode=0, n_origin_octaves=0,
                   n_dir_octaves=0, plucker=False):
        op = L.Op()
        op.kind = L.OP_RAY_ENCODE
        r = op.u.rays
        r.extrinsics, r.intrinsics, r.out_nchw, r.out_nhwc, r.img_map = ptr(extr), ptr(intr), ptr(out_nchw), ptr(out_nhwc), ptr(img_map)
        r.n_cam, r.h, r.w = extr.shape[0], h, w
        r.nhwc_c, r.nhwc_c_off, r.nhwc_dtype = (0, 0, L.F32) if out_nhwc is None else (out_nhwc.shape[-1], c_off, dt(out_nhwc))
        r.mode, r.n_origin_octaves, r.n_dir_octaves, r.plucker = mode, n_origin_octaves, n_dir_octaves, int(plucker)
        self._emit(op, name, 0.0, extr.shape[0] * h * w * 6 * 4.0, (extr, intr, out_nhwc, out_nchw, img_map))

    def posterior_sample(self, moments, noise, out, scale=1.0, name="posterior_sample"):
        n, c2, h, w = moments.shape
        op = L.Op()
        op.kind = L.OP_POSTERIOR_SAMPLE
        q = op.u.posterior
        q.moments, q.noise, q.out, q.n, q.c, q.hw, q.scale = ptr(moments), ptr(noise), ptr(out), n, c2 // 2, h * w, scale
        self._emit(op, name, 0.0, moments.numel() * 4 * 2.0, (moments, noise, out))
        return out

    def finalize(self, autotune: Optional[bool] = None) -> "Plan":
        assert self.record
        if autotune is None:
            autotune = os.environ.get("MVLDM_AUTOTUNE", "1") != "0"
        if autotune and torch.device(self.device).type == "cuda":
            autotune_igemm(self.ops, srcs=self.__dict__.get("_tune_srcs"), skinny=self._skinny_pw, keep=self.keep)
            autotune_wgrad(self.ops)
            if type(self) is Builder and _BATCH_SPLIT:
                self.ops, self.meta = autosplit_igemm(self.ops, self.meta, skinny=self._skinny_pw, keep=self.keep)
        return Plan(self.ops, self.meta, self.keep, self.device)


_TUNE_CACHE = {}
_WGRAD_CACHE = {}
_SPLIT_CACHE = {}
_VALIDATED = set()
_TUNE_TILES = tuple(int(t) for t in os.environ["MVLDM_TUNE_TILES"].split(",")) if os.environ.get("MVLDM_TUNE_TILES") else (0, 1, 2, 3, 4, 5, 6, 7, 8, 9, 10, 11, 12, 13, 14)


def tune_cache_state() -> dict:
    return {"version": 2, "igemm": {json.dumps(list(k)): (int(v) if isinstance(v, int) else list(v)) for k, v in _TUNE_CACHE.items()},
            "wgrad": {json.dumps(list(k)): int(v) for k, v in _WGRAD_CACHE.items()},
            "split": {json.dumps(list(k)): int(v) for k, v in _SPLIT_CACHE.items()}}


def set_tune_cache_state(state: dict, replace: bool = False) -> None:
    if replace:
        _TUNE_CACHE.clear()
        _WGRAD_CACHE.clear()
        _SPLIT_CACHE.clear()
    for name, cache in (("igemm", _TUNE_CACHE), ("wgrad", _WGRAD_CACHE), ("split", _SPLIT_CACHE)):
        for k, v in (state.get(name) or {}).items():
            cache[tuple(json.loads(k))] = int(v) if isinstance(v, int) else list(v)


def save_tune_cache(path: Optional[str] = None) -> Optional[str]:
    path = path or os.environ.get("MVLDM_TUNE_CACHE")
    if not path:
        return None
    tmp = f"{path}.{os.getpid()}.tmp"
    with open(tmp, "w") as f:
        json.dump(tune_cache_state(), f, indent=0, sort_keys=True)
    os.replace(tmp, path)
    return path


def load_tune_cache(path: Optional[str] = None) -> int:
    path = path or os.environ.get("MVLDM_TUNE_CACHE")
    if not path or not os.path.exists(path):
        return 0
    with open(path) as f:
        set_tune_cache_state(json.load(f))
    return len(_TUNE_CACHE) + len(_WGRAD_CACHE) + len(_SPLIT_CACHE)


def broadcast_tune_cache(dist, src: int = 0, device=None) -> None:
    box = [tune_cache_state() if dist.get_rank() == src else None]
    dist.broadcast_object_list(box, src=src, device=device)
    set_tune_cache_state(box[0], replace=True)


load_tune_cache()


def _igemm_signature(d) -> tuple:
    return (d.n_img, d.h_in, d.w_in, d.h_out, d.w_out, d.c0, d.c1, d.ksize, d.stride, d.pad, d.upsample, d.n_out, d.n_pad,
            d.k_pad, d.epilogue, d.act_dtype, d.dst_dtype, d.k_order, d.dst_ld, bool(d.residual), bool(d.row_bias),
            bool(d.bias), d.splitk, d.workspace_bytes)


_SMALL_ROWS = int(os.environ.get("MVLDM_TUNE_SMALL_ROWS", "64"))
_SPLITS = (0, 1, 2, 4, 8, 16, 32)
_MID_ROWS = int(os.environ.get("MVLDM_TUNE_MID_ROWS", "40000"))
_MID_SPLITS = (0, 1, 2, 3, 4, 6, 8)
_SMALL_TILES = tuple(int(t) for t in os.environ.get("MVLDM_TUNE_SMALL_TILES", "0,1,2,3,4,5").split(","))


_SKINNY = os.environ.get("MVLDM_SKINNY", "1") != "0"
_SKINNY_ROWS = int(os.environ.get("MVLDM_SKINNY_ROWS", "2304"))
_SKINNY_CFGS = tuple(int(c) for c in os.environ.get("MVLDM_SKINNY_CFGS", "0,1,2,5,6,7,8,9,10,12,13,18,19,20,38,39,40,41,42,43,44,46").split(","))


def skinny_rule(rows: int, n_pad: int) -> bool:
    if os.environ.get("MVLDM_AUTOTUNE", "1") != "0" or os.environ.get("MVLDM_SKINNY_RULE", "1") == "0":
        return False
    return rows <= 160 or (rows <= 1152 and n_pad <= 1280)


def skinny_candidate(pw: PackedWeight, rows: int, c0: int, c1: int, upsample, dtype) -> bool:
    return (_SKINNY and dtype != torch.float32 and rows <= _SKINNY_ROWS and not (upsample is True or upsample == 1) and pw.can_skinny()
            and c0 % 64 == 0 and c1 % 64 == 0)


def _unpack_choice(v):
    return (int(v), None) if isinstance(v, int) else (int(v[0]), None if v[1] is None else int(v[1]))


_TUNE_COLD = int(os.environ.get("MVLDM_TUNE_COLD", "9216"))
_THRASH = []
_THRASH_FILLS = [0]


def _thrash(device=None):
    if not _THRASH or (device is not None and _THRASH[0].device != torch.device(device)):
        _THRASH[:] = [torch.empty(640 << 20, dtype=torch.uint8, device=torch.cuda.current_device() if device is None else device)]
    return _THRASH[0]


def autotune_igemm(ops, min_rows: int = 2048, iters: int = 4, srcs=None, skinny=None, keep=None) -> int:
    lib = L.load()
    stream = torch.cuda.current_stream().cuda_stream
    e0, e1 = torch.cuda.Event(enable_timing=True), torch.cuda.Event(enable_timing=True)
    timed = 0
    tune_dev = next((t.device for pair in (srcs or {}).values() for t in pair if t is not None), None)
    if srcs:
        seen, gen = set(), None
        for pair in srcs.values():
            for t in pair:
                if t is not None and t.is_floating_point() and t.data_ptr() not in seen:
                    seen.add(t.data_ptr())
                    if gen is None:
                        gen = torch.Generator(device=t.device)
                        gen.manual_seed(0x5EED)
                    t.normal_(generator=gen)
    for idx, op in enumerate(ops):
        if op.kind != L.OP_IGEMM:
            continue
        d = op.u.igemm
        rows = d.n_img * d.h_out * d.w_out
        sk_pw = (skinny or {}).get(idx)
        if d.tile != 0 or d.act_dtype == L.F32 or d.k_order != 1 or (rows < min(min_rows, _SMALL_ROWS) and sk_pw is None):
            continue
        small = rows < min_rows
        key = _igemm_signature(d) + (("sk",) if sk_pw is not None else ())
        best = _TUNE_CACHE.get(key)
        if best is not None and (_unpack_choice(best)[0] & 63) not in (set(_TUNE_TILES) | set(_SMALL_TILES) | {17, 19} | ({15} if sk_pw is not None else set())):
            best = None
        if best is None:
            trial = L.Op()
            C.memmove(C.byref(trial), C.byref(op), C.sizeof(L.Op))
            can_split = small and bool(d.workspace) and d.splitk == 0
            mid = (not small) and rows < _MID_ROWS and bool(d.workspace) and d.splitk == 0
            cands = [(t, sk) for t in _TUNE_TILES for sk in _MID_SPLITS] if mid else [(t, None) for t in _TUNE_TILES] if not small else \
                    [(t, sk) for t in _SMALL_TILES if t in _TUNE_TILES or not os.environ.get("MVLDM_TUNE_TILES") for sk in (_SPLITS if can_split else (None,))]
            n_it = iters if not small else 3 * iters
            cold = _TUNE_COLD > 0 and rows <= _TUNE_COLD
            if not small and 17 not in _TUNE_TILES and not os.environ.get("MVLDM_TUNE_TILES") and d.ksize == 3 and d.stride == 1 \
                    and d.src1 is None and not d.upsample and d.w_in <= 24:
                cands = cands + [(17, None)]
            if not small and d.ksize == 1 and not os.environ.get("MVLDM_TUNE_TILES"):
                cands = cands + [(19, None), (13 | (1 << 13), None)]
            if sk_pw is not None:
                cands = cands + [(15 | (c << 8), 1) for c in _SKINNY_CFGS]
            results = []
            for tile, sk in cands:
                trial.u.igemm.tile = tile
                trial.u.igemm.splitk = d.splitk if sk is None else sk
                trial.u.igemm.weight, trial.u.igemm.k_order = d.weight, d.k_order
                if (tile & 63) == 15:
                    use_skinny(trial.u.igemm, sk_pw)
                if lib.mvldm_op_run(C.byref(trial), stream) != 0:
                    continue
                if cold:
                    t_sum = 0.0
                    for _ in range(n_it):
                        _thrash(tune_dev).zero_()
                        _THRASH_FILLS[0] += 1
                        e0.record()
                        lib.mvldm_op_run(C.byref(trial), stream)
                        e1.record()
                        e1.synchronize()
                        t_sum += e0.elapsed_time(e1)
                    results.append((t_sum, tile, sk))
                    continue
                e0.record()
                for _ in range(n_it):
                    lib.mvldm_op_run(C.byref(trial), stream)
                e1.record()
                e1.synchronize()
                results.append((e0.elapsed_time(e1), tile, sk))
            t_rule = next(t for t, tile, sk in results if tile == 0 and sk in (None, 0))
            t_best, tile_best, sk_best = min(results, key=lambda r: r[0])
            best = [tile_best, sk_best] if t_best < 0.97 * t_rule else [0, None]
            _TUNE_CACHE[key] = best
            _VALIDATED.add(key)
            timed += 1
        tile, sk = _unpack_choice(best)
        if tile != 0 and key not in _VALIDATED:
            trial = L.Op()
            C.memmove(C.byref(trial), C.byref(op), C.sizeof(L.Op))
            trial.u.igemm.tile = tile
            if sk is not None:
                trial.u.igemm.splitk = sk
            if (tile & 63) == 15:
                if sk_pw is None:
                    tile, sk = 0, None
                else:
                    use_skinny(trial.u.igemm, sk_pw)
            if tile != 0 and lib.mvldm_op_run(C.byref(trial), stream) != 0:
                tile, sk = 0, None
                _TUNE_CACHE[key] = [0, None]
            _VALIDATED.add(key)
        d.tile = tile
        if sk is not None:
            d.splitk = sk
        if (tile & 63) == 15:
            t = use_skinny(d, sk_pw)
            sk_pw._skinny_pinned = True
            if keep is not None:
                keep.append(t)
        elif sk_pw is not None:
            sk_pw.drop_skinny()
    if timed:
        save_tune_cache()
        _THRASH.clear()
    return timed


_BATCH_SPLIT = os.environ.get("MVLDM_BATCH_SPLIT", "1") != "0"
_SPLIT_MIN_ROWS = int(os.environ.get("MVLDM_BATCH_SPLIT_MIN_ROWS", "16384"))


def _split_candidates(d) -> list:
    rpi = d.h_out * d.w_out
    rows = d.n_img * rpi
    out = []
    for bn in (320, 256):
        n_tiles = -(-d.n_pad // bn)
        m_tiles = -(-rows // 256)
        if m_tiles * n_tiles <= 256 or (m_tiles * n_tiles) % 256 == 0 or (m_tiles * n_tiles) % 256 > 216:
            continue
        for m1 in range(m_tiles - 1, 0, -1):
            if (m1 * n_tiles) % 256 == 0 and (m1 * 256) % rpi == 0:
                n1 = m1 * 256 // rpi
                frac = 1.0 - n1 / d.n_img
                if 0.03 <= frac <= 0.45 and n1 not in out:
                    out.append(n1)
                break
    return out


def _image_range(op, i0: int, n: int):
    q = L.Op()
    C.memmove(C.byref(q), C.byref(op), C.sizeof(L.Op))
    d = q.u.igemm
    es = 4 if d.act_dtype == L.F32 else 2
    ds = 4 if d.dst_dtype == L.F32 else 2
    n_dst = d.n_out // 2 if d.epilogue == L.EPI_GEGLU else d.n_out
    px_in, px_out = d.h_in * d.w_in, d.h_out * d.w_out

    def off(p, nbytes):
        return (p + nbytes) if p else p
    d.src0 = off(d.src0, i0 * px_in * d.c0 * es)
    d.src1 = off(d.src1, i0 * px_in * d.c1 * es)
    d.dst = off(d.dst, i0 * px_out * (d.dst_ld or n_dst) * ds)
    d.residual = off(d.residual, i0 * px_out * n_dst * es)
    d.row_bias = off(d.row_bias, i0 * d.row_bias_ld * 4)
    d.n_img = n
    d.tile, d.splitk = 0, 0
    return q


def _time_ops(ops, iters: int) -> float:
    lib = L.load()
    stream = torch.cuda.current_stream().cuda_stream
    e0, e1 = torch.cuda.Event(enable_timing=True), torch.cuda.Event(enable_timing=True)
    for o in ops:
        L.check(lib.mvldm_op_run(C.byref(o), stream))
    e0.record()
    for _ in range(iters):
        for o in ops:
            lib.mvldm_op_run(C.byref(o), stream)
    e1.record()
    e1.synchronize()
    return e0.elapsed_time(e1) / iters


def autosplit_igemm(ops, meta, skinny=None, keep=None, iters: int = 6):
    new_ops, new_meta, decided = [], [], 0
    for idx, (op, m) in enumerate(zip(ops, meta)):
        d = op.u.igemm if op.kind == L.OP_IGEMM else None
        rows = d.n_img * d.h_out * d.w_out if d is not None else 0
        ok = (d is not None and rows >= _SPLIT_MIN_ROWS and d.act_dtype != L.F32 and d.k_order == 1 and d.stride == 1 and not d.upsample
              and (d.tile & 63) != 15 and not _PIN_TILE() and bool(d.workspace) and idx not in (skinny or {}))
        n1 = 0
        if ok:
            key = _igemm_signature(d)[:-2] + (d.workspace_bytes,)
            if key in _SPLIT_CACHE:
                n1 = _SPLIT_CACHE[key]
            else:
                best_t, t_whole = None, None
                for cand in _split_candidates(d):
                    parts = [_image_range(op, 0, cand), _image_range(op, cand, d.n_img - cand)]
                    try:
                        autotune_igemm(parts, iters=4)
                        if t_whole is None:
                            t_whole = _time_ops([op], iters)
                        t = _time_ops(parts, iters)
                    except L.MvldmError:
                        continue
                    if os.environ.get("MVLDM_BATCH_SPLIT_LOG"):
                        print(f"[batch split] {m.name}: {d.n_img} images x {d.h_out}x{d.w_out}, N {d.n_out}, K {d.k_pad}: whole {t_whole * 1e3:.1f} us (tile {d.tile & 63}, "
                              f"splitk {d.splitk}); {cand} + {d.n_img - cand}: {t * 1e3:.1f} us (tiles {parts[0].u.igemm.tile & 63} / {parts[1].u.igemm.tile & 63}, "
                              f"splitk {parts[1].u.igemm.splitk})", file=sys.stderr, flush=True)
                    if t < 0.97 * t_whole and (best_t is None or t < best_t):
                        best_t, n1 = t, cand
                _SPLIT_CACHE[key] = n1
                decided += 1
        if n1:
            parts = [_image_range(op, 0, n1), _image_range(op, n1, d.n_img - n1)]
            autotune_igemm(parts, iters=4)
            for k, (q, i0, cnt) in enumerate(zip(parts, (0, n1), (n1, d.n_img - n1))):
                q.tag = len(new_ops)
                new_ops.append(q)
                share = cnt / d.n_img
                new_meta.append(OpMeta(m.name if k == 0 else m.name + "[rest]", m.kind, m.flops * share, m.bytes * share))
        else:
            op.tag = len(new_ops)
            new_ops.append(op)
            new_meta.append(m)
    if decided:
        save_tune_cache()
    return new_ops, new_meta


_WGRAD_TARGETS = tuple(int(t) for t in os.environ.get("MVLDM_TUNE_WGRAD_TARGETS", "0,1,2,3,4,5").split(","))


def autotune_wgrad(ops, iters: int = 3) -> int:
    lib = L.load()
    stream = torch.cuda.current_stream().cuda_stream
    e0, e1 = torch.cuda.Event(enable_timing=True), torch.cuda.Event(enable_timing=True)
    timed = 0
    scratch = None
    for op in ops:
        if op.kind != L.OP_WGRAD:
            continue
        d = op.u.wgrad
        if d.act_dtype == L.F32 or (d.accumulate >> 8) & 3:
            continue
        key = (d.c0, d.c1, d.n_img, d.h_in, d.w_in, d.h_out, d.w_out, d.ksize, d.stride, d.pad, d.upsample, d.n_out, d.dy_ld, d.act_dtype,
               int(d.workspace_bytes), d.accumulate & 1)
        best = _WGRAD_CACHE.get(key)
        if best is None:
            trial = L.Op()
            C.memmove(C.byref(trial), C.byref(op), C.sizeof(L.Op))
            need = d.n_out * d.c_in * d.ksize * d.ksize
            if scratch is None or scratch.numel() < need:
                scratch = torch.zeros(need, dtype=torch.float32, device=torch.cuda.current_device())
            else:
                scratch[:need].zero_()
            trial.u.wgrad.grad = scratch.data_ptr()
            results = []
            for form in (1, 2):
                for tcode in _WGRAD_TARGETS:
                    v = form + 4 * tcode
                    trial.u.wgrad.accumulate = (d.accumulate & 1) | (v << 8)
                    if lib.mvldm_op_run(C.byref(trial), stream) != 0:
                        break
                    e0.record()
                    for _ in range(iters):
                        lib.mvldm_op_run(C.byref(trial), stream)
                    e1.record()
                    e1.synchronize()
                    results.append((e0.elapsed_time(e1), v))
            best = min(results)[1] if results else 0
            _WGRAD_CACHE[key] = best
            timed += 1
        d.accumulate = (d.accumulate & 1) | (best << 8)
    if timed:
        save_tune_cache()
    return timed


class Plan:

    def __init__(self, ops, meta, keep, device):
        self.meta, self._keep, self.device = list(meta), list(keep), device
        self.ops = list(ops)
        self.tiles = [int(op.u.igemm.tile) if op.kind == L.OP_IGEMM else None for op in ops]
        arr = (L.Op * max(len(ops), 1))(*ops)
        h = C.c_void_p()
        L.check(L.load().mvldm_plan_create(arr, len(ops), C.byref(h)))
        self._h = h
        self._stream = None
        self.captured = False

    def __len__(self):
        return len(self.meta)

    @staticmethod
    def _cur():
        return torch.cuda.current_stream().cuda_stream

    def run(self, first: int = 0, last: Optional[int] = None):
        last = len(self.meta) if last is None else last
        L.check(L.load().mvldm_plan_run_range(self._h, first, last, self._cur()))

    def capture(self):
        if self._stream is None:
            self._stream = torch.cuda.Stream(device=self.device)
        self._stream.wait_stream(torch.cuda.current_stream())
        L.check(L.load().mvldm_plan_capture(self._h, self._stream.cuda_stream))
        torch.cuda.current_stream().wait_stream(self._stream)
        self.captured = True

    def replay(self):
        L.check(L.load().mvldm_plan_replay(self._h, self._cur()))

    def profile(self, iters: int = 3):
        out = (C.c_float * max(len(self.meta), 1))()
        L.check(L.load().mvldm_plan_profile(self._h, self._cur(), iters, out))
        return [float(v) for v in out[:len(self.meta)]]

    def __del__(self):
        try:
            if getattr(self, "_h", None):
                L.load().mvldm_plan_destroy(self._h)
                self._h = None
        except Exception:
            pass
```

Measured before the change: 48.89.

## Add persistent wide-tile 3x3 conv kernel as autotune candidate

Adds a new persistent implicit-GEMM kernel for stride-1 3x3 convolutions (tile 20). It reuses the pipelined wide-N linear_pw machinery, which was factored into a shared pw_tile.h header, and loads the shifted im2col rows directly into LDS using per-tap boundary masks. The kernel supports bias, per-image row bias and residual, and it is registered as an autotuner candidate for large 3x3 convs. It is meant to cut per-tile launch and prologue overhead and to overlap loads with MFMA work. The risks are more code paths and constraints: n_pad must be a multiple of 320 and c0 a multiple of 64.

```diff
diff --git a/mv_ldm_amd/_build.py b/mv_ldm_amd/_build.py
--- a/mv_ldm_amd/_build.py
+++ b/mv_ldm_amd/_build.py
@@ -11,7 +11,7 @@
 CSRC = Path(__file__).resolve().parent / "csrc"
 LIB = CSRC / "libmvldm_hip.so"
 SOURCES = ["api.cpp", "plan.cpp", "igemm.hip", "igemm_small.hip", "igemm_large.hip", "igemm_xl.hip", "igemm_halo.hip", "pack.hip", "attention.hip", "norm.hip", "misc.hip",
-           "wgrad.hip", "attention_bwd.hip", "norm_bwd.hip", "train_misc.hip", "linear_pp.hip", "linear_pw.hip", "linear_ws.hip", "linear_rs.hip", "skinny.hip", "metrics.hip", "lpips.hip"]
+           "wgrad.hip", "attention_bwd.hip", "norm_bwd.hip", "train_misc.hip", "linear_pp.hip", "linear_pw.hip", "conv_pw.hip", "linear_ws.hip", "linear_rs.hip", "skinny.hip", "metrics.hip", "lpips.hip"]
 HEADERS = [*sorted(CSRC.glob("*.h")), CSRC.parent.parent / "include" / "mvldm.h"]
 FLAGS = ["--offload-arch=gfx950", "-O3", "-std=c++17", "-fPIC", "-ffp-contract=off", "-Wno-unused-result",
          "-Rpass-analysis=kernel-resource-usage"]
diff --git a/mv_ldm_amd/csrc/conv_pw.hip b/mv_ldm_amd/csrc/conv_pw.hip
--- /dev/null
+++ b/mv_ldm_amd/csrc/conv_pw.hip
@@ -0,0 +1,287 @@
+#include "pw_tile.h"
+
+namespace mvldm {
+
+struct ConvPWParams {
+    const void* a; const void* w; const float* bias; const float* row_bias; const void* residual; void* dst;
+    int M, K, c0, n_out, n_pad, n_dst, dst_ld, k_steps;
+    int h, wd, hw, row_bias_ld;
+    int tiles_m, tiles_n, m_per;
+    int gm, gn, nbn, wgx;
+    int spread;
+    float out_scale;
+    unsigned a_bytes, w_bytes, bias_bytes, rb_bytes, res_bytes, dst_bytes;
+    unsigned lead_bytes;
+};
+
+constexpr int CPW_TN = 5;
+
+struct ConvPwAddr {
+    unsigned a;
+    unsigned w;
+    unsigned m01, m23;
+    int n0;
+    bool valid;
+};
+
+template <int LO = 0, int HI = 1 << 20>
+__device__ __forceinline__ void cpw_issue_a(const ConvPWParams& p, char* smem, int slot, int wave, int cb, int t, const ConvPwAddr& ad) {
+    using G = PwGeo<CPW_TN>;
+    const __amdgpu_buffer_rsrc_t ra = __builtin_amdgcn_make_buffer_rsrc(const_cast<char*>(reinterpret_cast<const char*>(p.a)) - p.lead_bytes, 0,
+                                                                        p.a_bytes + p.lead_bytes, 0x00020000);
+    const int ty = (t >= 3) + (t >= 6), tx = t - 3 * ty;
+    const int soff = cb * 128 + (ty * p.wd + tx) * p.c0 * 2;
+    char* stage = smem + slot * G::STAGE;
+#pragma unroll
+    for (int it = (LO > 0 ? LO : 0); it < (HI < G::A_IT ? HI : G::A_IT); ++it) {
+        const unsigned mk = it < 2 ? ad.m01 : ad.m23;
+        const unsigned off = ((mk >> (t + 9 * (it & 1))) & 1u) ? ad.a : kBufOob;
+        __builtin_amdgcn_raw_ptr_buffer_load_lds(ra, (__attribute__((address_space(3))) void*)(stage + (wave + PW_NW * it) * 1024), 16, off,
+                                                 soff + it * 128 * p.c0, 0, 0);
+    }
+}
+template <int LO = 0, int HI = 1 << 20>
+__device__ __forceinline__ void cpw_issue_w(const ConvPWParams& p, char* smem, int slot, int wave, int ks, const ConvPwAddr& ad) {
+    using G = PwGeo<CPW_TN>;
+    const __amdgpu_buffer_rsrc_t rw = __builtin_amdgcn_make_buffer_rsrc(const_cast<void*>(p.w), 0, p.w_bytes, 0x00020000);
+    const int soff = ks * 128;
+    char* stage = smem + slot * G::STAGE + G::A_SLOT;
+#pragma unroll
+    for (int it = (LO > 0 ? LO : 0); it < (HI < G::W_IT ? HI : G::W_IT); ++it) {
+        const unsigned off = (ad.valid && ad.n0 + 64 * it < p.n_pad) ? ad.w : kBufOob;
+        __builtin_amdgcn_raw_ptr_buffer_load_lds(rw, (__attribute__((address_space(3))) void*)(stage + (wave + PW_NW * it) * 1024), 16, off,
+                                                 soff + it * 128 * p.K, 0, 0);
+    }
+}
+template <int LO, int HI>
+__device__ __forceinline__ void cpw_issue_group(const ConvPWParams& p, char* smem, int slot, int wave, int ks, int cb, int t, const ConvPwAddr& ad) {
+    using G = PwGeo<CPW_TN>;
+    if constexpr (LO < HI && LO < G::A_IT) cpw_issue_a<LO, HI>(p, smem, slot, wave, cb, t, ad);
+    if constexpr (LO < HI && HI > G::A_IT) cpw_issue_w<LO - G::A_IT, HI - G::A_IT>(p, smem, slot, wave, ks, ad);
+}
+
+__device__ __forceinline__ void cpw_offsets(const ConvPWParams& p, bool valid, int tm, int tn, int wave, int lane, ConvPwAddr& ad) {
+    using G = PwGeo<CPW_TN>;
+    const int slot = lane & 7, rsub = lane >> 3;
+    const int row = wave * 8 + rsub;
+    const unsigned chunk = (unsigned)((slot ^ ((row >> 1) & 7)) * 8);
+    const int m = tm * PW_BM + row, n = tn * G::BN + row;
+    ad.a = ((unsigned)m * (unsigned)p.c0 + chunk) * 2u;
+    ad.w = ((unsigned)n * (unsigned)p.K + chunk) * 2u;
+    ad.n0 = tn * G::BN;
+    ad.valid = valid;
+    unsigned mk[G::A_IT];
+#pragma unroll
+    for (int it = 0; it < G::A_IT; ++it) {
+        const unsigned mi = (unsigned)(m + 64 * it);
+        const unsigned img = mi / (unsigned)p.hw, rem = mi - img * (unsigned)p.hw;
+        const unsigned y = rem / (unsigned)p.wd, x = rem - y * (unsigned)p.wd;
+        const unsigned rowbits = (x > 0u ? 1u : 0u) | 2u | (x + 1u < (unsigned)p.wd ? 4u : 0u);
+        const unsigned all = (y > 0u ? rowbits : 0u) | (rowbits << 3) | (y + 1u < (unsigned)p.h ? rowbits << 6 : 0u);
+        mk[it] = (valid && mi < (unsigned)p.M) ? all : 0u;
+    }
+    static_assert(G::A_IT == 4, "two masks of two pieces");
+    ad.m01 = mk[0] | (mk[1] << 9);
+    ad.m23 = mk[2] | (mk[3] << 9);
+}
+
+__device__ __forceinline__ unsigned cpw_rb_off(const ConvPWParams& p, bool valid, int tm, int tn, int t) {
+    using G = PwGeo<CPW_TN>;
+    const int pc = tn * G::BN + 4 * t;
+    const unsigned img = (unsigned)(tm * PW_BM) / (unsigned)p.hw;
+    return (valid && 4 * t < G::BN && pc < p.n_out) ? (img * (unsigned)p.row_bias_ld + (unsigned)pc) * 4u : kBufOob;
+}
+__device__ __forceinline__ u32x4 cpw_load_rb(const ConvPWParams& p, unsigned off) {
+    const __amdgpu_buffer_rsrc_t rr = __builtin_amdgcn_make_buffer_rsrc(const_cast<float*>(p.row_bias), 0, p.rb_bytes, 0x00020000);
+    return __builtin_amdgcn_raw_buffer_load_b128(rr, off, 0, 0);
+}
+__device__ __forceinline__ u32x4 cpw_add_f32(const u32x4& x, const u32x4& y) {
+    u32x4 r;
+#pragma unroll
+    for (int e = 0; e < 4; ++e) r[e] = __float_as_uint(__uint_as_float(x[e]) + __uint_as_float(y[e]));
+    return r;
+}
+
+#define PW_STAMP()
+#define PW_GELU(x) (x)
+
+template <typename T, bool RES, bool ROWB, bool NT>
+__global__ __launch_bounds__(512) void conv_pw_kernel(const ConvPWParams p) {
+    constexpr int TN = CPW_TN, NOUT = TN;
+    constexpr bool GEGLU = false;
+    using G = PwGeo<TN>;
+    using Frag = typename LinMma<T>::Frag;
+    extern __shared__ __attribute__((aligned(16))) char smem[];
+    const int tid = threadIdx.x, lane = tid & 63;
+    const int wave = __builtin_amdgcn_readfirstlane(tid >> 6);
+    const int wm = wave >> 1, wn = wave & 1;
+    const int hi = lane >> 5, l31 = lane & 31;
+    const int prm = lin_perm(l31);
+
+    const int xcd = blockIdx.x & 7, lid = blockIdx.x >> 3;
+    const int m_lo = xcd * p.m_per, m_cnt = min(p.tiles_m, m_lo + p.m_per) - m_lo;
+    LinTileIter<ConvPWParams> cur, nxt, iss;
+    cur.set(p, 0, lid, m_lo, m_cnt);
+    if (!cur.valid) return;
+    nxt.set(p, cur.r + 1, lid, m_lo, m_cnt);
+    iss = cur;
+
+    u32x4 rdst;
+    rdst[0] = (unsigned)(uintptr_t)p.dst; rdst[1] = (unsigned)((uintptr_t)p.dst >> 32) & 0xFFFFu; rdst[2] = p.dst_bytes; rdst[3] = 0x00020000u;
+
+    const int a_off = (wm * 64 + l31) * 128 + ((hi ^ ((l31 >> 1) & 7)) << 4);
+    const int w_off = G::A_SLOT + (wn * 32 * TN + prm) * 128 + ((hi ^ ((prm >> 1) & 7)) << 4);
+
+    f32x16 acc[2][TN];
+    ConvPwAddr ad;
+    int ks_i = 1, cb_i = 0, t_i = 1;
+    const int kT = p.k_steps;
+
+    {
+        cpw_offsets(p, true, cur.tm, cur.tn, wave, lane, ad);
+#pragma unroll
+        for (int g = 0; g < 2; ++g) {
+            cpw_issue_a(p, smem, g, wave, 0, g, ad);
+            cpw_issue_w(p, smem, g, wave, g, ad);
+        }
+        u32x4 b = lin_load_bias<G::BN>(p, GEGLU, true, cur.tn, tid);
+        if constexpr (ROWB) b = cpw_add_f32(b, cpw_load_rb(p, cpw_rb_off(p, true, cur.tm, cur.tn, tid)));
+        __builtin_amdgcn_s_waitcnt(waitcnt_vmcnt(0));
+        if (4 * tid < G::BN) *reinterpret_cast<u32x4*>(smem + G::SLAB + tid * 16) = b;
+    }
+    int rs = 0;
+
+#define PW_ADVANCE()                                                                                              \
+    ++ks_i;                                                                                                       \
+    if (++t_i == 9) { t_i = 0; ++cb_i; }                                                                          \
+    if (ks_i == kT) {                                                                                             \
+        ks_i = 0; cb_i = 0;                                                                                       \
+        iss.set(p, iss.r + 1, lid, m_lo, m_cnt);                                                                  \
+        cpw_offsets(p, iss.valid, iss.tm, iss.tn, wave, lane, ad);                                                \
+    }
+#define PW_ISSUE(LO_, HI_, slot_) cpw_issue_group<LO_, HI_>(p, smem, slot_, wave, ks_i, cb_i, t_i, ad);
+#define PW_ISSUE_A(slot_) cpw_issue_a(p, smem, slot_, wave, cb_i, t_i, ad);
+#define PW_ISSUE_W(slot_) cpw_issue_w(p, smem, slot_, wave, ks_i, ad);
+#define PW_TOUCH(t_) false
+#define PW_TOUCH_ISSUE()
+#define PW_BIAS_READY(n_)                                                                                         \
+    if constexpr (ROWB) {                                                                                         \
+        asm volatile("s_waitcnt vmcnt(%1)" : "+v"(rbnext) : "n"(n_));                                             \
+        bnext = cpw_add_f32(bnext, rbnext);                                                                       \
+    }
+    bool pend = false;
+    const bool sp = p.spread != 0;
+    Frag fa0[2], fw0[TN], fa1[2], fw1[TN];
+    constexpr int kWaitLds = 0xC07F;
+    constexpr int kWaitFirst = waitcnt_vmcnt(4 * NOUT) & ~0x0F00;
+    constexpr int kWaitStepT = waitcnt_vmcnt(0) & ~0x0F00;
+    constexpr int kWaitStep1 = kWaitStepT;
+
+    for (; cur.valid; cur = nxt, nxt.set(p, nxt.r + 1, lid, m_lo, m_cnt)) {
+        __builtin_amdgcn_s_barrier();
+        {
+            const float* slab = reinterpret_cast<const float*>(smem + G::SLAB) + wn * 32 * TN + 8 * hi;
+#pragma unroll
+            for (int j = 0; j < TN; ++j)
+#pragma unroll
+                for (int a = 0; a < 4; ++a) {
+                    const f32x4 b = *reinterpret_cast<const f32x4*>(slab + 32 * j + 16 * (a >> 1) + 4 * (a & 1));
+#pragma unroll
+                    for (int e = 0; e < 4; ++e) { acc[0][j][4 * a + e] = b[e]; acc[1][j][4 * a + e] = b[e]; }
+                }
+        }
+        {
+            const char* st0 = smem + rs * G::STAGE;
+#pragma unroll
+            for (int i = 0; i < 2; ++i) fa0[i] = lin_frag<T>(st0 + a_off + i * 4096);
+#pragma unroll
+            for (int j = 0; j < TN; ++j) fw0[j] = lin_frag<T>(st0 + w_off + j * 4096);
+        }
+        PW_STEP(false, kWaitFirst, false, sp)
+#pragma unroll 1
+        for (int ks_t = 1; ks_t < kT - 1; ++ks_t) PW_STEP(false, kWaitStepT, false, sp && ks_t + 2 < kT)
+        u32x4 bnext, rbnext;
+        {
+            u32x4 rbias;
+            rbias[0] = (unsigned)(uintptr_t)p.bias; rbias[1] = (unsigned)((uintptr_t)p.bias >> 32) & 0xFFFFu; rbias[2] = p.bias_bytes; rbias[3] = 0x00020000u;
+            const int pc = nxt.tn * G::BN + 4 * tid;
+            const unsigned boff = (nxt.valid && 4 * tid < G::BN && pc < p.n_out) ? (unsigned)pc * 4u : kBufOob;
+            if constexpr (ROWB) {
+                u32x4 rrb;
+                rrb[0] = (unsigned)(uintptr_t)p.row_bias; rrb[1] = (unsigned)((uintptr_t)p.row_bias >> 32) & 0xFFFFu; rrb[2] = p.rb_bytes; rrb[3] = 0x00020000u;
+                const unsigned rboff = cpw_rb_off(p, nxt.valid, nxt.tm, nxt.tn, tid);
+                asm volatile("s_nop 4\n\tbuffer_load_dwordx4 %0, %2, %4, 0 offen\n\tbuffer_load_dwordx4 %1, %3, %5, 0 offen"
+                             : "=&v"(bnext), "=&v"(rbnext) : "v"(boff), "v"(rboff), "s"(rbias), "s"(rrb));
+            } else {
+                asm volatile("s_nop 4\n\tbuffer_load_dwordx4 %0, %1, %2, 0 offen" : "=v"(bnext) : "v"(boff), "s"(rbias));
+            }
+        }
+        PW_STEP(true, kWaitLds, false, false)
+#include "pw_epilogue.h"
+    }
+#undef PW_ADVANCE
+#undef PW_ISSUE
+#undef PW_ISSUE_A
+#undef PW_ISSUE_W
+#undef PW_TOUCH
+#undef PW_TOUCH_ISSUE
+#undef PW_BIAS_READY
+}
+
+bool conv_pw_applicable(const mvldm_igemm_desc& d) {
+    if (d.act_dtype == MVLDM_F32 || d.dst_dtype != d.act_dtype) return false;
+    if (d.ksize != 3 || d.stride != 1 || d.pad != 1 || d.upsample != 0 || d.k_order != 1 || d.splitk > 1) return false;
+    if (d.h_in != d.h_out || d.w_in != d.w_out || d.h_in < 1 || d.w_in < 1) return false;
+    if (d.epilogue != MVLDM_EPI_NONE) return false;
+    if (d.c1 != 0 || d.src1 != nullptr || d.c0 < 64 || d.c0 % 64 || d.k_pad != 9 * d.c0) return false;
+    if (d.n_pad % 320 || d.n_pad < d.n_out) return false;
+    const int n_dst = d.n_out;
+    const int dst_ld = d.dst_ld > 0 ? d.dst_ld : n_dst;
+    if (d.n_out % 8 || dst_ld % 8 || dst_ld < n_dst) return false;
+    if (d.row_bias && ((d.h_out * d.w_out) % PW_BM || ((uintptr_t)d.row_bias % 16) || d.row_bias_ld % 4 || d.row_bias_ld < d.n_out)) return false;
+    if (d.bias && ((uintptr_t)d.bias % 16)) return false;
+    if (((uintptr_t)d.dst % 16) || (d.residual && ((uintptr_t)d.residual % 16))) return false;
+    const double m = (double)d.n_img * d.h_out * d.w_out;
+    return m * d.c0 * 2.0 + (d.w_in + 1.0) * d.c0 * 2.0 < 4.0e9 && (double)d.n_pad * d.k_pad * 2.0 < 4.0e9 && m * dst_ld * 2.0 < 4.0e9 && m * n_dst * 2.0 < 4.0e9 &&
+           (double)d.n_img * d.row_bias_ld * 4.0 < 4.0e9;
+}
+
+template <typename T, bool RES, bool ROWB> static int conv_pw_launch(const ConvPWParams& p, int grid, hipStream_t s) {
+    static std::atomic<uint64_t> done{0};
+    if (int rc0 = ensure_dyn_smem(reinterpret_cast<const void*>(conv_pw_kernel<T, RES, ROWB, false>), PwGeo<CPW_TN>::SMEM, done)) return rc0;
+    hipLaunchKernelGGL((conv_pw_kernel<T, RES, ROWB, false>), dim3(grid), dim3(512), PwGeo<CPW_TN>::SMEM, s, p);
+    return check_launch();
+}
+
+int conv_pw_run(const mvldm_igemm_desc& d, hipStream_t s) {
+    MVLDM_REQUIRE(conv_pw_applicable(d), "igemm: tile 20 (persistent wide 3x3 conv) does not apply to this problem");
+    ConvPWParams p;
+    lin_fill_params(p, d, 0);
+    p.row_bias = d.row_bias; p.row_bias_ld = d.row_bias_ld;
+    p.rb_bytes = d.row_bias ? (unsigned)((double)d.n_img * d.row_bias_ld * 4.0) : 0u;
+    p.c0 = d.c0; p.K = 9 * d.c0; p.k_steps = p.K / 64;
+    p.h = d.h_in; p.wd = d.w_in; p.hw = d.h_in * d.w_in;
+    p.lead_bytes = (unsigned)(d.w_in + 1) * (unsigned)d.c0 * 2u;
+    constexpr int bn = 64 * CPW_TN;
+    const int cu_x = std::max(1, cu_count() / 8);
+    p.tiles_m = (p.M + PW_BM - 1) / PW_BM;
+    p.m_per = (p.tiles_m + 7) / 8;
+    p.tiles_n = d.n_pad / bn;
+    p.spread = !((d.tile >> 14) & 1);
+    p.wgx = std::min(cu_x, p.m_per * p.tiles_n);
+    lin_block_shape(p, 256.0 * d.c0 * 2.0, (double)bn * p.K * 2.0);
+    p.nbn = (p.tiles_n + p.gn - 1) / p.gn;
+    const int grid = 8 * p.wgx;
+    const bool res = d.residual != nullptr, rb = d.row_bias != nullptr;
+    return dispatch_dtype(d.act_dtype, [&](auto t) -> int {
+        using T = decltype(t);
+        if constexpr (sizeof(T) == 2) {
+            if (res) return rb ? conv_pw_launch<T, true, true>(p, grid, s) : conv_pw_launch<T, true, false>(p, grid, s);
+            return rb ? conv_pw_launch<T, false, true>(p, grid, s) : conv_pw_launch<T, false, false>(p, grid, s);
+        } else {
+            return set_error(MVLDM_ERR_ARG, "igemm: tile 20 needs a 16-bit activation type");
+        }
+    });
+}
+
+}
diff --git a/mv_ldm_amd/csrc/igemm.hip b/mv_ldm_amd/csrc/igemm.hip
--- a/mv_ldm_amd/csrc/igemm.hip
+++ b/mv_ldm_amd/csrc/igemm.hip
@@ -306,6 +306,7 @@
 int linear_ws_run(const mvldm_igemm_desc& d, hipStream_t s);
 int skinny_run(const mvldm_igemm_desc& d, hipStream_t s);
 int linear_rs_run(const mvldm_igemm_desc& d, hipStream_t s);
+int conv_pw_run(const mvldm_igemm_desc& d, hipStream_t s);
 
 int igemm_run(const mvldm_igemm_desc& d, hipStream_t s) {
     IgemmParams p;
@@ -313,6 +314,10 @@
     if (d.n_img == 0 || d.h_out == 0 || d.w_out == 0) return MVLDM_OK;
     const int req = d.tile & 63;
     if (req == 15) return skinny_run(d, s);
+    if (req == 20) {
+        MVLDM_REQUIRE(d.src0 && d.weight && d.dst, "igemm: null pointer");
+        return conv_pw_run(d, s);
+    }
     if (req == 12 || req == 13 || req == 14 || req == 19) {
         MVLDM_REQUIRE(d.src0 && d.weight && d.dst, "igemm: null pointer");
         return req == 12 ? linear_pp_run(d, s) : req == 13 ? linear_pw_run(d, s) : req == 14 ? linear_ws_run(d, s) : linear_rs_run(d, s);
diff --git a/mv_ldm_amd/csrc/linear_pw.hip b/mv_ldm_amd/csrc/linear_pw.hip
--- a/mv_ldm_amd/csrc/linear_pw.hip
+++ b/mv_ldm_amd/csrc/linear_pw.hip
@@ -1,6 +1,6 @@
 #include <cstdlib>
 
-#include "linear_common.h"
+#include "pw_tile.h"
 
 namespace mvldm {
 
@@ -33,24 +33,6 @@
 #define PW_GELU(x) gelu_erf_16(x)
 #endif
 
-constexpr int PW_BM = 256, PW_NW = 8;
-#ifndef PW_SP3
-#define PW_SP3 4
-#define PW_SP0 3
-#define PW_SP1 2
-#endif
-
-template <int TN> struct PwGeo {
-    static constexpr int BN = 64 * TN;
-    static constexpr int A_SLOT = PW_BM * 128, W_SLOT = BN * 128, STAGE = A_SLOT + W_SLOT;
-    static constexpr int A_IT = PW_BM / 8 / PW_NW;
-    static constexpr int W_IT = BN / 8 / PW_NW;
-    static constexpr int P = A_IT + W_IT;
-    static constexpr int Q0 = PW_SP3 < P ? PW_SP3 : P, Q1 = Q0 + PW_SP0 < P ? Q0 + PW_SP0 : P, Q2 = Q1 + PW_SP1 < P ? Q1 + PW_SP1 : P;
-    static constexpr int RING = 2 * STAGE;
-    static constexpr int SLAB = RING;
-    static constexpr int SMEM = SLAB + 2048;
-};
 
 struct PwAddr {
     unsigned a0, a1;
@@ -140,43 +122,6 @@
     return (valid && 4 * t < G::BN && pc < p.n_out) ? (unsigned)oc * 4u : kBufOob;
 }
 
-template <bool NT>
-__device__ __forceinline__ void pw_store2(const u32x4& rdst, const u32x4& d0, unsigned o0, const u32x4& d1, unsigned o1) {
-    if constexpr (NT)
-        asm volatile("s_nop 4\n\tbuffer_store_dwordx4 %0, %1, %4, 0 offen nt\n\tbuffer_store_dwordx4 %2, %3, %4, 0 offen nt\n\ts_nop 2"
-                     ::"v"(d0), "v"(o0), "v"(d1), "v"(o1), "s"(rdst) : "memory");
-    else
-        asm volatile("s_nop 4\n\tbuffer_store_dwordx4 %0, %1, %4, 0 offen\n\tbuffer_store_dwordx4 %2, %3, %4, 0 offen\n\ts_nop 2"
-                     ::"v"(d0), "v"(o0), "v"(d1), "v"(o1), "s"(rdst) : "memory");
-}
-
-template <int CTRL> __device__ __forceinline__ u32x4 pw_qperm(const u32x4& v) {
-    u32x4 r;
-#pragma unroll
-    for (int c = 0; c < 4; ++c) r[c] = (unsigned)__builtin_amdgcn_update_dpp(0, (int)v[c], CTRL, 0xF, 0xF, true);
-    return r;
-}
-__device__ __forceinline__ u32x4 pw_sel(bool take_a, const u32x4& a, const u32x4& b) {
-    u32x4 r;
-#pragma unroll
-    for (int c = 0; c < 4; ++c) r[c] = take_a ? a[c] : b[c];
-    return r;
-}
-__device__ __forceinline__ void pw_quad_transpose(u32x4& c0, u32x4& c1, u32x4& c2, u32x4& c3, bool odd, bool upper) {
-    constexpr int X1 = 0xB1, X2 = 0x4E;
-    const u32x4 x0 = pw_sel(odd, pw_qperm<X1>(c1), c0), x1 = pw_sel(odd, c1, pw_qperm<X1>(c0));
-    const u32x4 x2 = pw_sel(odd, pw_qperm<X1>(c3), c2), x3 = pw_sel(odd, c3, pw_qperm<X1>(c2));
-    c0 = pw_sel(upper, pw_qperm<X2>(x2), x0);
-    c2 = pw_sel(upper, x2, pw_qperm<X2>(x0));
-    c1 = pw_sel(upper, pw_qperm<X2>(x3), x1);
-    c3 = pw_sel(upper, x3, pw_qperm<X2>(x1));
-}
-__device__ __forceinline__ unsigned pw_line_off(int M, int tm, int wm, int i, int j, int half, int l31, int hi, int col0, int ld, int n_dst) {
-    const int t = 2 * (j & 1) + half, k = l31 & 3;
-    const int m = tm * PW_BM + wm * 64 + i * 32 + (l31 & ~3) + t;
-    const int col = col0 + 32 * (j & ~1) + 8 * (2 * k + hi);
-    return (m < M && col < n_dst) ? ((unsigned)m * (unsigned)ld + (unsigned)col) * 2u : kBufOob;
-}
 
 template <typename T, int TN, int EPI, bool RES, bool NT>
 __global__ __launch_bounds__(512) void linear_pw_kernel(const LinPWParams p) {
@@ -232,62 +177,23 @@
     int tr_n = 0;
 #endif
 
-#define PW_SUB(ca_, cw_, na_, nw_, NEXT_, nslot_, nkk_, MODE_, SPN_)                                              \
-    {                                                                                                             \
-        const char* st_ = smem + (nslot_) * G::STAGE;                                                             \
-        const int ao_ = a_off ^ ((nkk_) << 5), wo_ = w_off ^ ((nkk_) << 5);                                       \
-        if (NEXT_) {                                                                                              \
-            na_[0] = lin_frag<T>(st_ + ao_);                                                                      \
-            na_[1] = lin_frag<T>(st_ + ao_ + 4096);                                                               \
-            nw_[0] = lin_frag<T>(st_ + wo_);                                                                      \
-        }                                                                                                         \
-        _Pragma("unroll") for (int j = 0; j < TN; ++j) {                                                          \
-            __builtin_amdgcn_sched_barrier(0);                                                                    \
-            acc[0][j] = LinMma<T>::mma(cw_[j], ca_[0], acc[0][j]);                                                \
-            acc[1][j] = LinMma<T>::mma(cw_[j], ca_[1], acc[1][j]);                                                \
-            if (NEXT_ && j + 1 < TN) nw_[j + 1] = lin_frag<T>(st_ + wo_ + (j + 1) * 4096);                        \
-            if ((MODE_) == 1 && j == 0) {                                                                         \
-                if (++ks_i == kT) {                                                                               \
-                    ks_i = 0;                                                                                     \
-                    iss.set(p, iss.r + 1, lid, m_lo, m_cnt);                                                  \
-                    pw_offsets<TN>(p, iss.valid, iss.tm, iss.tn, wave, lane, ad);                                 \
-                }                                                                                                 \
-                if (SPN_) pw_issue_group<TN, 0, G::Q0>(p, smem, rs, wave, lane, ks_i, ad);                        \
-                else pw_issue_a<TN>(p, smem, rs, wave, lane, ks_i, ad);                                           \
-            }                                                                                                     \
-            if ((MODE_) == 1 && j == 2 && !(SPN_)) pw_issue_w<TN>(p, smem, rs, wave, ks_i, ad);                   \
-            if ((MODE_) == 2 && j == 1 && pend) pw_issue_group<TN, G::Q0, G::Q1>(p, smem, rs ^ 1, wave, lane, ks_i, ad); \
-            if ((MODE_) == 3 && j == 1 && pend) pw_issue_group<TN, G::Q1, G::Q2>(p, smem, rs ^ 1, wave, lane, ks_i, ad); \
-            if ((MODE_) == 4 && j == 1 && pend) pw_issue_group<TN, G::Q2, G::P>(p, smem, rs ^ 1, wave, lane, ks_i, ad);  \
-        }                                                                                                         \
-        __builtin_amdgcn_sched_barrier(0);                                                                        \
-    }
-#define PW_STEP(LAST_, WAIT_, TOUCH_, SPN_)                                                                       \
-    {                                                                                                             \
-        PW_STAMP()                                                                                                \
-        if ((TOUCH_) && p.touch) {                                                                                \
-             \
-            const int kt_ = ks_t + PW_TOUCH_AHEAD;                                                                \
-            const bool own_ = kt_ < kT;                                                                           \
-            pw_touch_a<TN>(p, smem, wave, lane, __builtin_amdgcn_readfirstlane(own_ ? cur.tm : nxt.tm),           \
-                           __builtin_amdgcn_readfirstlane(own_ ? kt_ : kt_ - kT), own_ || nxt.valid);             \
-        }                                                                                                         \
-        PW_SUB(fa0, fw0, fa1, fw1, true, rs, 1, 2, false)                                                         \
-        PW_SUB(fa1, fw1, fa0, fw0, true, rs, 2, 3, false)                                                         \
-        PW_SUB(fa0, fw0, fa1, fw1, true, rs, 3, 4, false)                                                         \
-        PW_STAMP()                                                                                                \
-        if ((TOUCH_) && p.touch) __builtin_amdgcn_s_waitcnt(kWaitStep1);                                          \
-        else __builtin_amdgcn_s_waitcnt(WAIT_);                                                                   \
-        PW_STAMP()                                                                                                \
-        __builtin_amdgcn_s_barrier();                                                                             \
-        PW_STAMP()                                                                                                \
-        {                                                                                                         \
-            const bool spn_ = (SPN_);                                                                             \
-            PW_SUB(fa1, fw1, fa0, fw0, !(LAST_), rs ^ 1, 0, 1, spn_)                                              \
-            pend = spn_;                                                                                          \
-        }                                                                                                         \
-        rs ^= 1;                                                                                                  \
-    }
+#define PW_ADVANCE()                                                                                              \
+    if (++ks_i == kT) {                                                                                           \
+        ks_i = 0;                                                                                                 \
+        iss.set(p, iss.r + 1, lid, m_lo, m_cnt);                                                                  \
+        pw_offsets<TN>(p, iss.valid, iss.tm, iss.tn, wave, lane, ad);                                             \
+    }
+#define PW_ISSUE(LO_, HI_, slot_) pw_issue_group<TN, LO_, HI_>(p, smem, slot_, wave, lane, ks_i, ad);
+#define PW_ISSUE_A(slot_) pw_issue_a<TN>(p, smem, slot_, wave, lane, ks_i, ad);
+#define PW_ISSUE_W(slot_) pw_issue_w<TN>(p, smem, slot_, wave, ks_i, ad);
+#define PW_TOUCH(t_) ((t_) && p.touch)
+#define PW_BIAS_READY(n_)
+#define PW_TOUCH_ISSUE()                                                                                          \
+     \
+    const int kt_ = ks_t + PW_TOUCH_AHEAD;                                                                        \
+    const bool own_ = kt_ < kT;                                                                                   \
+    pw_touch_a<TN>(p, smem, wave, lane, __builtin_amdgcn_readfirstlane(own_ ? cur.tm : nxt.tm),                   \
+                   __builtin_amdgcn_readfirstlane(own_ ? kt_ : kt_ - kT), own_ || nxt.valid);
     bool pend = false;
     const bool sp = p.spread && !p.touch && kT >= 4;
     Frag fa0[2], fw0[TN], fa1[2], fw1[TN];
@@ -329,100 +235,7 @@
         }
         { const int ks_t = 0; PW_STEP(true, kWaitLds, false, false) }
         PW_STAMP()
-        {
-            const int col0 = GEGLU ? (cur.tn * G::BN + wn * 32 * TN) >> 1 : cur.tn * G::BN + wn * 32 * TN;
-            const bool q_odd = (l31 & 1) != 0, q_upper = (l31 & 2) != 0;
-            unsigned row_dst[2], row_res[2];
-#pragma unroll
-            for (int i = 0; i < 2; ++i) {
-                const int m = cur.tm * PW_BM + wm * 64 + i * 32 + l31;
-                row_dst[i] = m < p.M ? (unsigned)m * (unsigned)p.dst_ld * 2u : kLinRowNone;
-                row_res[i] = m < p.M ? (unsigned)m * (unsigned)p.n_dst * 2u : kLinRowNone;
-            }
-            u32x4 out[2][NOUT][2];
-            if constexpr (RES) {
-                constexpr int NB = 2 * TN;
-                u32x4 rres;
-                rres[0] = (unsigned)(uintptr_t)p.residual; rres[1] = (unsigned)((uintptr_t)p.residual >> 32) & 0xFFFFu; rres[2] = p.res_bytes; rres[3] = 0x00020000u;
-                u32x4 r[NB][2];
-#define PW_RES_OFFS(b_)                                                                                                         \
-        const bool pair_ = (((b_) % TN) | 1) < TN;                                                                              \
-        const unsigned o0_ = pair_ ? pw_line_off(p.M, cur.tm, wm, (b_) / TN, (b_) % TN, 0, l31, hi, col0, p.n_dst, p.n_dst)     \
-                                   : lin_off(row_res[(b_) / TN], col0 + 32 * ((b_) % TN) + 8 * hi, p.n_dst);                    \
-        const unsigned o1_ = pair_ ? pw_line_off(p.M, cur.tm, wm, (b_) / TN, (b_) % TN, 1, l31, hi, col0, p.n_dst, p.n_dst)     \
-                                   : lin_off(row_res[(b_) / TN], col0 + 32 * ((b_) % TN) + 16 + 8 * hi, p.n_dst);
-#define PW_RES_ISSUE(b_)                                                                                                        \
-    if constexpr ((b_) < NB) {                                                                                                  \
-        PW_RES_OFFS(b_)                                                                                                         \
-        asm volatile("s_nop 4\n\tbuffer_load_dwordx4 %0, %2, %4, 0 offen\n\tbuffer_load_dwordx4 %1, %3, %4, 0 offen"             \
-                     : "=&v"(r[(b_) < NB ? (b_) : 0][0]), "=&v"(r[(b_) < NB ? (b_) : 0][1]) : "v"(o0_), "v"(o1_), "s"(rres));   \
-    }
-#define PW_RES_BLOCK(b_)                                                                                                        \
-    if constexpr ((b_) < NB) {                                                                                                  \
-        constexpr int i_ = (b_) / TN, j_ = (b_) % TN;                                                                           \
-        constexpr int left_ = NB - 1 - (b_) < PW_D - 1 ? NB - 1 - (b_) : PW_D - 1;                                              \
-        if constexpr ((b_) == 0) {                                                                                              \
-            asm volatile("s_waitcnt vmcnt(%3)" : "+v"(r[0][0]), "+v"(r[0][1]), "+v"(bnext) : "n"(2 * left_));                  \
-            if (4 * tid < G::BN) *reinterpret_cast<u32x4*>(smem + G::SLAB + tid * 16) = bnext;                                  \
-        } else {                                                                                                                \
-            asm volatile("s_waitcnt vmcnt(%2)" : "+v"(r[(b_) < NB ? (b_) : 0][0]), "+v"(r[(b_) < NB ? (b_) : 0][1]) : "n"(2 * left_)); \
-        }                                                                                                                       \
-        constexpr bool paired_ = (j_ | 1) < TN;                                                                                 \
-        if constexpr (!paired_) {                                                                                               \
-            float c_[16];                                                                                                       \
-            _Pragma("unroll") for (int k = 0; k < 16; ++k) c_[k] = acc[i_][j_][k];                                              \
-            lin_pack<T, true>(c_, p.out_scale, r[(b_) < NB ? (b_) : 0], out[i_][j_]);                                           \
-        } else if constexpr ((j_ & 1) == 1) {                                                                                   \
-                \
-            constexpr int bp_ = (b_) > 0 ? (b_) - 1 : 0;                                                                        \
-            pw_quad_transpose(r[bp_][0], r[bp_][1], r[(b_) < NB ? (b_) : 0][0], r[(b_) < NB ? (b_) : 0][1], q_odd, q_upper);    \
-            float c_[16];                                                                                                       \
-            _Pragma("unroll") for (int k = 0; k < 16; ++k) c_[k] = acc[i_][j_ - 1][k];                                          \
-            lin_pack<T, true>(c_, p.out_scale, r[bp_], out[i_][j_ - 1]);                                                        \
-            _Pragma("unroll") for (int k = 0; k < 16; ++k) c_[k] = acc[i_][j_][k];                                              \
-            lin_pack<T, true>(c_, p.out_scale, r[(b_) < NB ? (b_) : 0], out[i_][j_]);                                           \
-            pw_quad_transpose(out[i_][j_ - 1][0], out[i_][j_ - 1][1], out[i_][j_][0], out[i_][j_][1], q_odd, q_upper);          \
-        }                                                                                                                       \
-        PW_RES_ISSUE((b_) + PW_D)                                                                                               \
-    }
-                constexpr int PW_D = 4;
-                PW_RES_ISSUE(0) PW_RES_ISSUE(1) PW_RES_ISSUE(2) PW_RES_ISSUE(3)
-                PW_RES_BLOCK(0) PW_RES_BLOCK(1) PW_RES_BLOCK(2) PW_RES_BLOCK(3) PW_RES_BLOCK(4)
-                PW_RES_BLOCK(5) PW_RES_BLOCK(6) PW_RES_BLOCK(7) PW_RES_BLOCK(8) PW_RES_BLOCK(9)
-                static_assert(NB <= 10, "blocks listed above");
-#undef PW_RES_ISSUE
-#undef PW_RES_BLOCK
-            } else {
-                asm volatile("s_waitcnt vmcnt(%1)" : "+v"(bnext) : "n"(G::P));
-                if (4 * tid < G::BN) *reinterpret_cast<u32x4*>(smem + G::SLAB + tid * 16) = bnext;
-#pragma unroll
-                for (int i = 0; i < 2; ++i)
-#pragma unroll
-                    for (int j = 0; j < NOUT; ++j) {
-                        float c[16];
-                        if constexpr (GEGLU) {
-#pragma unroll
-                            for (int k = 0; k < 16; ++k) c[k] = acc[i][2 * j][k] * PW_GELU(acc[i][2 * j + 1][k]);
-                        } else {
-#pragma unroll
-                            for (int k = 0; k < 16; ++k) c[k] = acc[i][j][k];
-                        }
-                        const u32x4 none[2] = {u32x4{0u, 0u, 0u, 0u}, u32x4{0u, 0u, 0u, 0u}};
-                        lin_pack<T, false>(c, p.out_scale, none, out[i][j]);
-                        if ((j & 1) == 1) pw_quad_transpose(out[i][j - 1][0], out[i][j - 1][1], out[i][j][0], out[i][j][1], q_odd, q_upper);
-                    }
-            }
-#pragma unroll
-            for (int i = 0; i < 2; ++i)
-#pragma unroll
-                for (int j = 0; j < NOUT; ++j)
-                    if ((j | 1) < NOUT)
-                        pw_store2<NT>(rdst, out[i][j][0], pw_line_off(p.M, cur.tm, wm, i, j, 0, l31, hi, col0, p.dst_ld, p.n_dst), out[i][j][1],
-                                      pw_line_off(p.M, cur.tm, wm, i, j, 1, l31, hi, col0, p.dst_ld, p.n_dst));
-                    else
-                        pw_store2<NT>(rdst, out[i][j][0], lin_off(row_dst[i], col0 + 32 * j + 8 * hi, p.n_dst), out[i][j][1],
-                                      lin_off(row_dst[i], col0 + 32 * j + 16 + 8 * hi, p.n_dst));
-        }
+#include "pw_epilogue.h"
     }
 #ifdef MVLDM_PW_TRACE
     if (tr_on) {
@@ -431,8 +244,13 @@
         for (int i = lane; i < 192; i += 64) p.trace[i] = i < tr_n ? reinterpret_cast<const unsigned*>(smem + G::SLAB + 1280)[i] : 0u;
     }
 #endif
-#undef PW_SUB
-#undef PW_STEP
+#undef PW_ADVANCE
+#undef PW_ISSUE
+#undef PW_ISSUE_A
+#undef PW_ISSUE_W
+#undef PW_TOUCH
+#undef PW_TOUCH_ISSUE
+#undef PW_BIAS_READY
 }
 
 bool linear_pw_applicable(const mvldm_igemm_desc& d) {
diff --git a/mv_ldm_amd/csrc/pw_epilogue.h b/mv_ldm_amd/csrc/pw_epilogue.h
--- /dev/null
+++ b/mv_ldm_amd/csrc/pw_epilogue.h
@@ -0,0 +1,96 @@
+        {
+            const int col0 = GEGLU ? (cur.tn * G::BN + wn * 32 * TN) >> 1 : cur.tn * G::BN + wn * 32 * TN;
+            const bool q_odd = (l31 & 1) != 0, q_upper = (l31 & 2) != 0;
+            unsigned row_dst[2], row_res[2];
+#pragma unroll
+            for (int i = 0; i < 2; ++i) {
+                const int m = cur.tm * PW_BM + wm * 64 + i * 32 + l31;
+                row_dst[i] = m < p.M ? (unsigned)m * (unsigned)p.dst_ld * 2u : kLinRowNone;
+                row_res[i] = m < p.M ? (unsigned)m * (unsigned)p.n_dst * 2u : kLinRowNone;
+            }
+            u32x4 out[2][NOUT][2];
+            if constexpr (RES) {
+                constexpr int NB = 2 * TN;
+                u32x4 rres;
+                rres[0] = (unsigned)(uintptr_t)p.residual; rres[1] = (unsigned)((uintptr_t)p.residual >> 32) & 0xFFFFu; rres[2] = p.res_bytes; rres[3] = 0x00020000u;
+                u32x4 r[NB][2];
+#define PW_RES_OFFS(b_)                                                                                                         \
+        const bool pair_ = (((b_) % TN) | 1) < TN;                                                                              \
+        const unsigned o0_ = pair_ ? pw_line_off(p.M, cur.tm, wm, (b_) / TN, (b_) % TN, 0, l31, hi, col0, p.n_dst, p.n_dst)     \
+                                   : lin_off(row_res[(b_) / TN], col0 + 32 * ((b_) % TN) + 8 * hi, p.n_dst);                    \
+        const unsigned o1_ = pair_ ? pw_line_off(p.M, cur.tm, wm, (b_) / TN, (b_) % TN, 1, l31, hi, col0, p.n_dst, p.n_dst)     \
+                                   : lin_off(row_res[(b_) / TN], col0 + 32 * ((b_) % TN) + 16 + 8 * hi, p.n_dst);
+#define PW_RES_ISSUE(b_)                                                                                                        \
+    if constexpr ((b_) < NB) {                                                                                                  \
+        PW_RES_OFFS(b_)                                                                                                         \
+        asm volatile("s_nop 4\n\tbuffer_load_dwordx4 %0, %2, %4, 0 offen\n\tbuffer_load_dwordx4 %1, %3, %4, 0 offen"             \
+                     : "=&v"(r[(b_) < NB ? (b_) : 0][0]), "=&v"(r[(b_) < NB ? (b_) : 0][1]) : "v"(o0_), "v"(o1_), "s"(rres));   \
+    }
+#define PW_RES_BLOCK(b_)                                                                                                        \
+    if constexpr ((b_) < NB) {                                                                                                  \
+        constexpr int i_ = (b_) / TN, j_ = (b_) % TN;                                                                           \
+        constexpr int left_ = NB - 1 - (b_) < PW_D - 1 ? NB - 1 - (b_) : PW_D - 1;                                              \
+        if constexpr ((b_) == 0) {                                                                                              \
+            asm volatile("s_waitcnt vmcnt(%3)" : "+v"(r[0][0]), "+v"(r[0][1]), "+v"(bnext) : "n"(2 * left_));                  \
+            PW_BIAS_READY(2 * left_)                                                                                            \
+            if (4 * tid < G::BN) *reinterpret_cast<u32x4*>(smem + G::SLAB + tid * 16) = bnext;                                  \
+        } else {                                                                                                                \
+            asm volatile("s_waitcnt vmcnt(%2)" : "+v"(r[(b_) < NB ? (b_) : 0][0]), "+v"(r[(b_) < NB ? (b_) : 0][1]) : "n"(2 * left_)); \
+        }                                                                                                                       \
+        constexpr bool paired_ = (j_ | 1) < TN;                                                                                 \
+        if constexpr (!paired_) {                                                                                               \
+            float c_[16];                                                                                                       \
+            _Pragma("unroll") for (int k = 0; k < 16; ++k) c_[k] = acc[i_][j_][k];                                              \
+            lin_pack<T, true>(c_, p.out_scale, r[(b_) < NB ? (b_) : 0], out[i_][j_]);                                           \
+        } else if constexpr ((j_ & 1) == 1) {                                                                                   \
+                \
+            constexpr int bp_ = (b_) > 0 ? (b_) - 1 : 0;                                                                        \
+            pw_quad_transpose(r[bp_][0], r[bp_][1], r[(b_) < NB ? (b_) : 0][0], r[(b_) < NB ? (b_) : 0][1], q_odd, q_upper);    \
+            float c_[16];                                                                                                       \
+            _Pragma("unroll") for (int k = 0; k < 16; ++k) c_[k] = acc[i_][j_ - 1][k];                                          \
+            lin_pack<T, true>(c_, p.out_scale, r[bp_], out[i_][j_ - 1]);                                                        \
+            _Pragma("unroll") for (int k = 0; k < 16; ++k) c_[k] = acc[i_][j_][k];                                              \
+            lin_pack<T, true>(c_, p.out_scale, r[(b_) < NB ? (b_) : 0], out[i_][j_]);                                           \
+            pw_quad_transpose(out[i_][j_ - 1][0], out[i_][j_ - 1][1], out[i_][j_][0], out[i_][j_][1], q_odd, q_upper);          \
+        }                                                                                                                       \
+        PW_RES_ISSUE((b_) + PW_D)                                                                                               \
+    }
+                constexpr int PW_D = 4;
+                PW_RES_ISSUE(0) PW_RES_ISSUE(1) PW_RES_ISSUE(2) PW_RES_ISSUE(3)
+                PW_RES_BLOCK(0) PW_RES_BLOCK(1) PW_RES_BLOCK(2) PW_RES_BLOCK(3) PW_RES_BLOCK(4)
+                PW_RES_BLOCK(5) PW_RES_BLOCK(6) PW_RES_BLOCK(7) PW_RES_BLOCK(8) PW_RES_BLOCK(9)
+                static_assert(NB <= 10, "blocks listed above");
+#undef PW_RES_ISSUE
+#undef PW_RES_BLOCK
+            } else {
+                asm volatile("s_waitcnt vmcnt(%1)" : "+v"(bnext) : "n"(G::P));
+                PW_BIAS_READY(G::P)
+                if (4 * tid < G::BN) *reinterpret_cast<u32x4*>(smem + G::SLAB + tid * 16) = bnext;
+#pragma unroll
+                for (int i = 0; i < 2; ++i)
+#pragma unroll
+                    for (int j = 0; j < NOUT; ++j) {
+                        float c[16];
+                        if constexpr (GEGLU) {
+#pragma unroll
+                            for (int k = 0; k < 16; ++k) c[k] = acc[i][2 * j][k] * PW_GELU(acc[i][2 * j + 1][k]);
+                        } else {
+#pragma unroll
+                            for (int k = 0; k < 16; ++k) c[k] = acc[i][j][k];
+                        }
+                        const u32x4 none[2] = {u32x4{0u, 0u, 0u, 0u}, u32x4{0u, 0u, 0u, 0u}};
+                        lin_pack<T, false>(c, p.out_scale, none, out[i][j]);
+                        if ((j & 1) == 1) pw_quad_transpose(out[i][j - 1][0], out[i][j - 1][1], out[i][j][0], out[i][j][1], q_odd, q_upper);
+                    }
+            }
+#pragma unroll
+            for (int i = 0; i < 2; ++i)
+#pragma unroll
+                for (int j = 0; j < NOUT; ++j)
+                    if ((j | 1) < NOUT)
+                        pw_store2<NT>(rdst, out[i][j][0], pw_line_off(p.M, cur.tm, wm, i, j, 0, l31, hi, col0, p.dst_ld, p.n_dst), out[i][j][1],
+                                      pw_line_off(p.M, cur.tm, wm, i, j, 1, l31, hi, col0, p.dst_ld, p.n_dst));
+                    else
+                        pw_store2<NT>(rdst, out[i][j][0], lin_off(row_dst[i], col0 + 32 * j + 8 * hi, p.n_dst), out[i][j][1],
+                                      lin_off(row_dst[i], col0 + 32 * j + 16 + 8 * hi, p.n_dst));
+        }
diff --git a/mv_ldm_amd/csrc/pw_tile.h b/mv_ldm_amd/csrc/pw_tile.h
--- /dev/null
+++ b/mv_ldm_amd/csrc/pw_tile.h
@@ -0,0 +1,112 @@
+#pragma once
+#include "linear_common.h"
+
+namespace mvldm {
+
+constexpr int PW_BM = 256, PW_NW = 8;
+#ifndef PW_SP3
+#define PW_SP3 4
+#define PW_SP0 3
+#define PW_SP1 2
+#endif
+
+template <int TN> struct PwGeo {
+    static constexpr int BN = 64 * TN;
+    static constexpr int A_SLOT = PW_BM * 128, W_SLOT = BN * 128, STAGE = A_SLOT + W_SLOT;
+    static constexpr int A_IT = PW_BM / 8 / PW_NW;
+    static constexpr int W_IT = BN / 8 / PW_NW;
+    static constexpr int P = A_IT + W_IT;
+    static constexpr int Q0 = PW_SP3 < P ? PW_SP3 : P, Q1 = Q0 + PW_SP0 < P ? Q0 + PW_SP0 : P, Q2 = Q1 + PW_SP1 < P ? Q1 + PW_SP1 : P;
+    static constexpr int RING = 2 * STAGE;
+    static constexpr int SLAB = RING;
+    static constexpr int SMEM = SLAB + 2048;
+};
+
+template <bool NT>
+__device__ __forceinline__ void pw_store2(const u32x4& rdst, const u32x4& d0, unsigned o0, const u32x4& d1, unsigned o1) {
+    if constexpr (NT)
+        asm volatile("s_nop 4\n\tbuffer_store_dwordx4 %0, %1, %4, 0 offen nt\n\tbuffer_store_dwordx4 %2, %3, %4, 0 offen nt\n\ts_nop 2"
+                     ::"v"(d0), "v"(o0), "v"(d1), "v"(o1), "s"(rdst) : "memory");
+    else
+        asm volatile("s_nop 4\n\tbuffer_store_dwordx4 %0, %1, %4, 0 offen\n\tbuffer_store_dwordx4 %2, %3, %4, 0 offen\n\ts_nop 2"
+                     ::"v"(d0), "v"(o0), "v"(d1), "v"(o1), "s"(rdst) : "memory");
+}
+
+template <int CTRL> __device__ __forceinline__ u32x4 pw_qperm(const u32x4& v) {
+    u32x4 r;
+#pragma unroll
+    for (int c = 0; c < 4; ++c) r[c] = (unsigned)__builtin_amdgcn_update_dpp(0, (int)v[c], CTRL, 0xF, 0xF, true);
+    return r;
+}
+__device__ __forceinline__ u32x4 pw_sel(bool take_a, const u32x4& a, const u32x4& b) {
+    u32x4 r;
+#pragma unroll
+    for (int c = 0; c < 4; ++c) r[c] = take_a ? a[c] : b[c];
+    return r;
+}
+__device__ __forceinline__ void pw_quad_transpose(u32x4& c0, u32x4& c1, u32x4& c2, u32x4& c3, bool odd, bool upper) {
+    constexpr int X1 = 0xB1, X2 = 0x4E;
+    const u32x4 x0 = pw_sel(odd, pw_qperm<X1>(c1), c0), x1 = pw_sel(odd, c1, pw_qperm<X1>(c0));
+    const u32x4 x2 = pw_sel(odd, pw_qperm<X1>(c3), c2), x3 = pw_sel(odd, c3, pw_qperm<X1>(c2));
+    c0 = pw_sel(upper, pw_qperm<X2>(x2), x0);
+    c2 = pw_sel(upper, x2, pw_qperm<X2>(x0));
+    c1 = pw_sel(upper, pw_qperm<X2>(x3), x1);
+    c3 = pw_sel(upper, x3, pw_qperm<X2>(x1));
+}
+__device__ __forceinline__ unsigned pw_line_off(int M, int tm, int wm, int i, int j, int half, int l31, int hi, int col0, int ld, int n_dst) {
+    const int t = 2 * (j & 1) + half, k = l31 & 3;
+    const int m = tm * PW_BM + wm * 64 + i * 32 + (l31 & ~3) + t;
+    const int col = col0 + 32 * (j & ~1) + 8 * (2 * k + hi);
+    return (m < M && col < n_dst) ? ((unsigned)m * (unsigned)ld + (unsigned)col) * 2u : kBufOob;
+}
+
+#define PW_SUB(ca_, cw_, na_, nw_, NEXT_, nslot_, nkk_, MODE_, SPN_)                                              \
+    {                                                                                                             \
+        const char* st_ = smem + (nslot_) * G::STAGE;                                                             \
+        const int ao_ = a_off ^ ((nkk_) << 5), wo_ = w_off ^ ((nkk_) << 5);                                       \
+        if (NEXT_) {                                                                                              \
+            na_[0] = lin_frag<T>(st_ + ao_);                                                                      \
+            na_[1] = lin_frag<T>(st_ + ao_ + 4096);                                                               \
+            nw_[0] = lin_frag<T>(st_ + wo_);                                                                      \
+        }                                                                                                         \
+        _Pragma("unroll") for (int j = 0; j < TN; ++j) {                                                          \
+            __builtin_amdgcn_sched_barrier(0);                                                                    \
+            acc[0][j] = LinMma<T>::mma(cw_[j], ca_[0], acc[0][j]);                                                \
+            acc[1][j] = LinMma<T>::mma(cw_[j], ca_[1], acc[1][j]);                                                \
+            if (NEXT_ && j + 1 < TN) nw_[j + 1] = lin_frag<T>(st_ + wo_ + (j + 1) * 4096);                        \
+            if ((MODE_) == 1 && j == 0) {                                                                         \
+                PW_ADVANCE()                                                                                      \
+                if (SPN_) PW_ISSUE(0, G::Q0, rs)                                                                  \
+                else PW_ISSUE_A(rs)                                                                               \
+            }                                                                                                     \
+            if ((MODE_) == 1 && j == 2 && !(SPN_)) PW_ISSUE_W(rs)                                                 \
+            if ((MODE_) == 2 && j == 1 && pend) PW_ISSUE(G::Q0, G::Q1, rs ^ 1)                                    \
+            if ((MODE_) == 3 && j == 1 && pend) PW_ISSUE(G::Q1, G::Q2, rs ^ 1)                                    \
+            if ((MODE_) == 4 && j == 1 && pend) PW_ISSUE(G::Q2, G::P, rs ^ 1)                                     \
+        }                                                                                                         \
+        __builtin_amdgcn_sched_barrier(0);                                                                        \
+    }
+#define PW_STEP(LAST_, WAIT_, TOUCH_, SPN_)                                                                       \
+    {                                                                                                             \
+        PW_STAMP()                                                                                                \
+        if (PW_TOUCH(TOUCH_)) {                                                                                   \
+            PW_TOUCH_ISSUE()                                                                                      \
+        }                                                                                                         \
+        PW_SUB(fa0, fw0, fa1, fw1, true, rs, 1, 2, false)                                                         \
+        PW_SUB(fa1, fw1, fa0, fw0, true, rs, 2, 3, false)                                                         \
+        PW_SUB(fa0, fw0, fa1, fw1, true, rs, 3, 4, false)                                                         \
+        PW_STAMP()                                                                                                \
+        if (PW_TOUCH(TOUCH_)) __builtin_amdgcn_s_waitcnt(kWaitStep1);                                             \
+        else __builtin_amdgcn_s_waitcnt(WAIT_);                                                                   \
+        PW_STAMP()                                                                                                \
+        __builtin_amdgcn_s_barrier();                                                                             \
+        PW_STAMP()                                                                                                \
+        {                                                                                                         \
+            const bool spn_ = (SPN_);                                                                             \
+            PW_SUB(fa1, fw1, fa0, fw0, !(LAST_), rs ^ 1, 0, 1, spn_)                                              \
+            pend = spn_;                                                                                          \
+        }                                                                                                         \
+        rs ^= 1;                                                                                                  \
+    }
+
+}
diff --git a/mv_ldm_amd/plan.py b/mv_ldm_amd/plan.py
--- a/mv_ldm_amd/plan.py
+++ b/mv_ldm_amd/plan.py
@@ -519,7 +519,7 @@
         small = rows < min_rows
         key = _igemm_signature(d) + (("sk",) if sk_pw is not None else ())
         best = _TUNE_CACHE.get(key)
-        if best is not None and (_unpack_choice(best)[0] & 63) not in (set(_TUNE_TILES) | set(_SMALL_TILES) | {17, 19} | ({15} if sk_pw is not None else set())):
+        if best is not None and (_unpack_choice(best)[0] & 63) not in (set(_TUNE_TILES) | set(_SMALL_TILES) | {17, 19, 20} | ({15} if sk_pw is not None else set())):
             best = None
         if best is None:
             trial = L.Op()
@@ -533,6 +533,8 @@
             if not small and 17 not in _TUNE_TILES and not os.environ.get("MVLDM_TUNE_TILES") and d.ksize == 3 and d.stride == 1 \
                     and d.src1 is None and not d.upsample and d.w_in <= 24:
                 cands = cands + [(17, None)]
+            if not small and d.ksize == 3 and d.stride == 1 and d.src1 is None and not d.upsample and not os.environ.get("MVLDM_TUNE_TILES"):
+                cands = cands + [(20, None)]
             if not small and d.ksize == 1 and not os.environ.get("MVLDM_TUNE_TILES"):
                 cands = cands + [(19, None), (13 | (1 << 13), None)]
             if sk_pw is not None:
```

After: 48.97, median of 6. No clear change (+0.2%).
